# afiaka87/clip-guided-diffusion

Measured on AMD Instinct MI355X. Metric: diffusion steps/sec (UNet+CLIP+grad) at 256x256 cutn=16, higher is better.
Workload: dtype bf16x3 (split-bf16 MFMA, fp32 accumulate, fp32 storage); 1 GPU; BASELINE configs[1]: 256x256 class-cond UNet (554M), respace 250, cutn 16, batch 1/GPU, CLIP ViT-B/32, cgs 1000 tv 150 range 50, randomize_class, p_sample; global_batch=1, world_size_checked=1, collectives=none (single process)

## Files before the change

### clip-guided-diffusion_amd/csrc/capi.hip

```cpp
#include "../../include/cgd_mi355x.h"
#include "common.h"
#include "guidance.h"
#include "kernels.h"
#include "mfma_stage.h"

#define S(stream) ((hipStream_t)(stream))

extern "C" {

const char* cgd_version(void) { return "cgd_mi355x 0.1 (gfx950)"; }

int cgd_ctx_create(cgd_ctx** out, int device) {
  if (!out) return -3;
  cgd_ctx* ctx = new cgd_ctx();
  ctx->device = device;
  int prev = -1;
  (void)hipGetDevice(&prev);
  if (hipSetDevice(device) != hipSuccess) {
    delete ctx;
    return -1;
  }
  struct Restore {
    int d;
    ~Restore() {
      if (d >= 0) (void)hipSetDevice(d);
    }
  } restore{prev};
  hipDeviceProp_t prop;
  if (hipGetDeviceProperties(&prop, device) == hipSuccess) {
    ctx->num_cu = prop.multiProcessorCount;
    if (std::string(prop.gcnArchName).find("gfx950") == std::string::npos) {
      fprintf(stderr, "cgd_mi355x: device %d is %s, this library is built for gfx950 only\n", device, prop.gcnArchName);
      delete ctx;
      return -4;
    }
  }
  if (const char* e = getenv("CGD_DEFER")) ctx->defer_mode = atoi(e);
  if (const char* e = getenv("CGD_HGEMM_VAR")) ctx->hgemm_var = atoi(e);
  if (const char* e = getenv("CGD_HGEMM_EPI")) ctx->hgemm_epi = atoi(e);
  if (const char* e = getenv("CGD_TILE_ORDER")) ctx->tile_order = atoi(e);
  if (const char* e = getenv("CGD_FUSE_GN")) sscanf(e, "%d,%d,%d,%d", &ctx->fuse_gn, &ctx->fuse_gn_max_m, &ctx->fuse_gn_min_m, &ctx->fuse_gn_skip_m);
  if (const char* e = getenv("CGD_FUSE_ACT")) ctx->fuse_act = atoi(e);
  if (const char* e = getenv("CGD_HCONV_W8")) ctx->hconv_w8 = atoi(e);
  if (const char* e = getenv("CGD_ATTN_X3")) ctx->attn_x3 = atoi(e);
  if (const char* e = getenv("CGD_ATTN_FLASH")) ctx->attn_flash = atoi(e);
  int wino_env_mode = -1;
  if (const char* e = getenv("CGD_WINO")) sscanf(e, "%d,%d", &wino_env_mode, &ctx->wino_min_m);
  if (const char* e = getenv("CGD_THIN")) ctx->thin_direct = atoi(e);
  if (const char* e = getenv("CGD_GEMV")) ctx->gemv_mode = atoi(e);
  if (const char* e = getenv("CGD_WINO_NC")) ctx->wino_nc = atoi(e);
  ctx->wino_nc_default = ctx->wino_nc;
  if (wino_env_mode >= 0) cgd_apply_wino_mode(ctx, wino_env_mode);
  if (const char* e = getenv("CGD_GN_EPI")) ctx->gn_epi = atoi(e);
  if (const char* e = getenv("CGD_HGEMM_KG")) ctx->hgemm_kg = atoi(e) < 0 || atoi(e) > 2 ? 1 : atoi(e);
  if (const char* e = getenv("CGD_HGEMM_TM96")) ctx->hgemm_tm96 = atoi(e);
  if (const char* e = getenv("CGD_NT")) ctx->weight_nt = atoi(e);
  if (const char* e = getenv("CGD_KGEMM")) sscanf(e, "%d,%d,%d,%d,%d", &ctx->kgemm_mode, &ctx->kgemm_max_m, &ctx->kgemm_var, &ctx->kgemm_big_m, &ctx->kgemm_big_n);
  if (const char* e = getenv("CGD_EMBED_FUSE")) ctx->embed_fuse = atoi(e);
  if (const char* e = getenv("CGD_KCONV")) sscanf(e, "%d,%d,%d,%d,%d,%d,%d", &ctx->kconv_mode, &ctx->kconv_max_m, &ctx->kconv_min_chunks, &ctx->kconv_tw8, &ctx->kconv_slots, &ctx->kconv_ring, &ctx->kconv_th16);
  if (const char* e = getenv("CGD_HCONV_SPLIT")) sscanf(e, "%d,%d", &ctx->hconv_slots, &ctx->hconv_min_chunks);
  if (ctx->kconv_min_chunks < 1) ctx->kconv_min_chunks = 1;
  if (ctx->hconv_min_chunks < 1) ctx->hconv_min_chunks = 1;
  if (const char* e = getenv("CGD_HCONV_SMALL")) sscanf(e, "%d,%d,%d", &ctx->hconv_small_m, &ctx->hconv_small_slots, &ctx->hconv_small_min_chunks);
  ctx->ws_bytes = (size_t)256 << 20;
  if (hipMalloc((void**)&ctx->ws, ctx->ws_bytes) != hipSuccess) {
    delete ctx;
    return -1;
  }
  *out = ctx;
  return 0;
}

void cgd_ctx_destroy(cgd_ctx* ctx) {
  if (!ctx) return;
  {
  DeviceScope dev_scope(ctx);
  if (ctx->ws) (void)hipFree(ctx->ws);
  cgd_frag_cache_clear(ctx);
  cgd_chanstats_clear(ctx);
  if (ctx->frag_tmp) (void)hipFree(ctx->frag_tmp);
  for (ProfRec& r : ctx->prof_recs) {
    (void)hipEventDestroy(r.a);
    (void)hipEventDestroy(r.b);
  }
  for (hipEvent_t e : ctx->prof_pool) (void)hipEventDestroy(e);
  }
  delete ctx;
}

const char* cgd_last_error(cgd_ctx* ctx) { return ctx ? ctx->err.c_str() : "null context"; }

#define CGD_NEED_CTX(ctx)   \
  if (!(ctx)) return -3;    \
  DeviceScope dev_scope__(ctx)

int cgd_set_precision(cgd_ctx* ctx, int mode) {
  CGD_NEED_CTX(ctx);
  if (mode < 0 || mode > 2) CGD_FAIL(ctx, "precision mode must be 0 (f32), 1 (bf16x3) or 2 (bf16)");
  ctx->precision = mode;
  return 0;
}
int cgd_get_precision(cgd_ctx* ctx) { return ctx ? ctx->precision : -3; }
int64_t cgd_ctx_device_allocs(cgd_ctx* ctx) { return ctx ? (int64_t)ctx->device_allocs : -3; }

int cgd_set_tiles(cgd_ctx* ctx, int large, int small) {
  CGD_NEED_CTX(ctx);
  ctx->tile_huge = large >= 1000000 ? large / 1000000 : ctx->tile_huge;
  ctx->tile_large = large % 1000000;
  ctx->tile_small = small;
  return 0;
}

int cgd_set_hgemm(cgd_ctx* ctx, int mode, int min_m, int min_chunks) {
  CGD_NEED_CTX(ctx);
  ctx->hgemm_mode = mode;
  if (min_m > 0) ctx->hgemm_min_m = min_m;
  if (min_chunks > 0) ctx->hgemm_min_chunks = min_chunks;
  return 0;
}

int cgd_profile(cgd_ctx* ctx, int enable) {
  CGD_NEED_CTX(ctx);
  ctx->prof_on = enable != 0;
  return 0;
}
// ... 259 lines not shown
namespace {
__global__ __launch_bounds__(256) void mfma_peak_kernel(float* out, int iters) {
  cgd_f32x16 acc[4];
  for (int a = 0; a < 4; ++a)
    for (int e = 0; e < 16; ++e) acc[a][e] = 0.f;
  cgd_bf16x8 x, y;
  for (int e = 0; e < 8; ++e) {
    x[e] = (__bf16)(float)((threadIdx.x * 7 + e) % 13 - 6);
    y[e] = (__bf16)(0.001f * (float)((threadIdx.x * 3 + e) % 11 - 5));
  }
  for (int it = 0; it < iters; ++it) {
#pragma unroll
    for (int r = 0; r < 3; ++r)
#pragma unroll
      for (int a = 0; a < 4; ++a) acc[a] = __builtin_amdgcn_mfma_f32_32x32x16_bf16(x, y, acc[a], 0, 0, 0);
  }
  float s = 0.f;
  for (int a = 0; a < 4; ++a)
    for (int e = 0; e < 16; ++e) s += acc[a][e];
  if (s == 12345.678f) out[blockIdx.x * blockDim.x + threadIdx.x] = s;
}
}
extern "C" {
int cgd_op_mfma_peak(cgd_ctx* ctx, int iters, double* flop_out, void* stream) {
  CGD_NEED_CTX(ctx);
  if (iters <= 0) CGD_FAIL(ctx, "cgd_op_mfma_peak: iters must be positive");
  const int blocks = ctx->num_cu;
  if (flop_out) *flop_out = 2.0 * 32 * 32 * 16 * 12.0 * iters * blocks * 4;
  CGD_LAUNCH(mfma_peak_kernel, dim3(blocks), dim3(256), 0, S(stream), ctx->ws, iters);
  CGD_HIP(ctx, hipGetLastError());
  return 0;
}
int cgd_op_new_pass(cgd_ctx* ctx) {
  CGD_NEED_CTX(ctx);
  ++ctx->stats_serial;
  return 0;
}
int64_t cgd_op_gn_stats_offset(int B, int HW, int C) { return (int64_t)cgd_gn_stats_offset(B, HW, C); }
int64_t cgd_op_gn_record_merges(cgd_ctx* ctx) { return ctx ? (int64_t)ctx->gn_record_merges : -3; }
int cgd_set_wino(cgd_ctx* ctx, int mode, int min_m) {
  CGD_NEED_CTX(ctx);
  if (mode < 0 || (mode > 3 && mode != 5)) CGD_FAIL(ctx, "cgd_set_wino: mode must be 0, 1, 2, 3 or 5");
  cgd_apply_wino_mode(ctx, mode);
  if (min_m > 0) ctx->wino_min_m = min_m;
  return 0;
}
int cgd_set_hconv(cgd_ctx* ctx, int mode, int min_m) {
  CGD_NEED_CTX(ctx);
  ctx->hconv_mode = mode & 15;
  ctx->hconv_var = mode >> 4;
  ctx->hconv_min_m = min_m;
  return 0;
}
int cgd_op_conv3x3(cgd_ctx* ctx, const float* x, int ldx, const float* w, const float* w_frag, float* y, int ldy, const float* bias,
                   const float* R, int ldr, int Bn, int H, int W, int Cin, int Cout, int ups, int force_tile, int splitk, void* stream) {
  CGD_NEED_CTX(ctx);
  GemmParams p;
  p.Bpk = w_frag;
  p.A = x; p.lda = ldx; p.B = w; p.ldb = 9 * Cin; p.C = y; p.ldc = ldy; p.bias = bias; p.R = R; p.ldr = ldr;
  p.M = Bn * H * W; p.N = Cout; p.conv = 1; p.H = H; p.W = W; p.Cin = Cin; p.ups = ups; p.force_tile = force_tile; p.splitk = splitk;
  return cgd_launch_gemm(ctx, p, S(stream));
}
int cgd_op_conv_in(cgd_ctx* ctx, const float* x, const float* w, const float* bias, float* y, int Bn, int H, int W, int Cin, int Cout,
                   void* stream) {
  CGD_NEED_CTX(ctx);
  return cgd_launch_conv_in(ctx, x, w, bias, y, Bn, H, W, Cin, Cout, S(stream));
}
int cgd_op_conv_thin_out(cgd_ctx* ctx, const float* x, int ldx, const float* w, const float* bias, float* y, int Bn, int H, int W,
                         int Cin, int Cout, void* stream) {
  CGD_NEED_CTX(ctx);
  return cgd_launch_conv_thin_out(ctx, x, ldx, w, bias, y, Bn, H, W, Cin, Cout, S(stream));
}
int64_t cgd_op_gn_scratch_floats(int B, int HW, int C) { return (int64_t)cgd_gn_scratch_floats(B, HW, C); }
int cgd_op_gn_fwd(cgd_ctx* ctx, const float* x, int ldx, float* y, int ldy, int B, int HW, int C, const float* gamma, const float* beta,
                  const float* film, int act, float eps, float* scratch, void* stream) {
  CGD_NEED_CTX(ctx);
  return cgd_launch_gn_fwd(ctx, x, ldx, y, ldy, B, HW, C, gamma, beta, film, 2 * C, act, eps, scratch, S(stream));
}
int cgd_op_gn_bwd(cgd_ctx* ctx, const float* x, int ldx, const float* dz, int lddz, float* dx, int lddx, const float* add, int ldadd,
                  int B, int HW, int C, int act, float* scratch, void* stream) {
  CGD_NEED_CTX(ctx);
  return cgd_launch_gn_bwd(ctx, x, ldx, dz, lddz, dx, lddx, add, ldadd, B, HW, C, act, scratch, S(stream));
}
int cgd_op_ln_fwd(cgd_ctx* ctx, const float* x, float* y, int rows, int C, const float* gamma, const float* beta, float eps, float* stats,
                  void* stream) {
  CGD_NEED_CTX(ctx);
  return cgd_launch_ln_fwd(ctx, x, C, y, C, rows, C, gamma, beta, eps, stats, S(stream));
}
int cgd_op_ln_bwd(cgd_ctx* ctx, const float* x, const float* dy, float* dx, int rows, int C, const float* gamma, const float* stats,
                  void* stream) {
  CGD_NEED_CTX(ctx);
  return cgd_launch_ln_bwd(ctx, x, C, dy, C, dx, C, nullptr, 0, rows, C, gamma, stats, S(stream));
}
int cgd_op_pool2x2(cgd_ctx* ctx, const float* in, float* out, int B, int Ho, int Wo, int C, float scale, void* stream) {
  CGD_NEED_CTX(ctx);
  return cgd_launch_pool2x2(ctx, in, C, out, C, nullptr, 0, B, Ho, Wo, C, scale, S(stream));
}
int cgd_op_upsample2x(cgd_ctx* ctx, const float* in, float* out, int B, int Ho, int Wo, int C, float scale, void* stream) {
  CGD_NEED_CTX(ctx);
  return cgd_launch_upsample2x(ctx, in, C, out, C, nullptr, 0, B, Ho, Wo, C, scale, S(stream));
}
int cgd_op_act(cgd_ctx* ctx, const float* x, const float* dy, float* out, int64_t n, int act, void* stream) {
  CGD_NEED_CTX(ctx);
  if (dy) return cgd_launch_act_bwd(ctx, x, dy, out, n, act, S(stream));
  return cgd_launch_act_fwd(ctx, x, out, n, act, S(stream));
}
int64_t cgd_op_attn_buf_floats(int nb, int heads, int T, int d, int which) {
  const int64_t Tp = attn_tp(T), C = (int64_t)heads * d;
  switch (which) {
    case 0: return (int64_t)nb * 3 * C * Tp;
    case 4: return (int64_t)nb * C * Tp;
    default: return (int64_t)nb * heads * T * Tp;
  }
}
int cgd_op_attn_fwd(cgd_ctx* ctx, const float* qkv, float* out, int nb, int heads, int T, int d, int legacy, float* bufs[5],
                    void* stream) {
  CGD_NEED_CTX(ctx);
  AttnShape sh{nb, heads, T, d, heads * d, legacy};
  AttnBufs bf{bufs[0], bufs[1], bufs[2], bufs[3], bufs[4]};
  return cgd_attn_fwd(ctx, sh, qkv, 3 * heads * d, out, heads * d, bf, S(stream));
}
int cgd_op_attn_fwd_causal(cgd_ctx* ctx, const float* qkv, float* out, int nb, int heads, int T, int d, float* bufs[5], void* stream) {
  CGD_NEED_CTX(ctx);
  AttnShape sh{nb, heads, T, d, heads * d, 0, 1};
  AttnBufs bf{bufs[0], bufs[1], bufs[2], bufs[3], bufs[4]};
  return cgd_attn_fwd(ctx, sh, qkv, 3 * heads * d, out, heads * d, bf, S(stream));
}
int cgd_op_attn_bwd(cgd_ctx* ctx, const float* qkv, const float* dout, float* dqkv, int nb, int heads, int T, int d, int legacy,
                    float* bufs[5], void* stream) {
  CGD_NEED_CTX(ctx);
  AttnShape sh{nb, heads, T, d, heads * d, legacy};
  AttnBufs bf{bufs[0], bufs[1], bufs[2], bufs[3], bufs[4]};
  return cgd_attn_bwd(ctx, sh, qkv, 3 * heads * d, dout, heads * d, dqkv, 3 * heads * d, bf, S(stream));
}
}

void cgd_apply_wino_mode(cgd_ctx* ctx, int mode) {
  if (mode < 0 || (mode > 3 && mode != 5)) mode = 1;
  ctx->wino_mode = mode == 5 ? 3 : mode;
  ctx->wino_nc = mode == 5 ? 3 : ctx->wino_nc_default;
}
```

### clip-guided-diffusion_amd/csrc/common.h

```cpp
#pragma once
#include <hip/hip_runtime.h>
#include <stdint.h>
#include <stdio.h>
#include <atomic>
#include <string>
#include <utility>
#include <vector>

inline std::atomic<unsigned long long> g_cgd_launches{0}, g_cgd_reduces{0};
#define CGD_LAUNCH(...)                                          \
  do {                                                           \
    g_cgd_launches.fetch_add(1, std::memory_order_relaxed);      \
    hipLaunchKernelGGL(__VA_ARGS__);                             \
  } while (0)

enum { CGD_PREC_F32 = 0, CGD_PREC_BF16X3 = 1, CGD_PREC_BF16 = 2 };

enum { CGD_PROF_GEMM = 0, CGD_PROF_HCONV = 1, CGD_PROF_GN = 2, CGD_PROF_WCONV = 3, CGD_PROF_KCONV = 4, CGD_PROF_WCONV_GNB = 5, CGD_PROF_KINDS = 6 };

struct ProfRec {
  hipEvent_t a = nullptr, b = nullptr;
  double flops = 0.0;
  int kind = 0;
  bool live = false;
};

struct SplitSrc {
  const float* ws = nullptr;
  const float* bias = nullptr;
  const float* R = nullptr;
  long stride = 0;
  int n = 0;
  int N = 0, ldr = 0;
  float alpha = 1.f;
};
struct PendingReduce {
  bool valid = false;
  SplitSrc src;
  float* C = nullptr;
  int ldc = 0, M = 0;
  hipStream_t stream = nullptr;
};

struct ChanStatsEntry {
  const float* C = nullptr;
  int ldc = 0, N = 0;
  long M = 0;
  float* buf = nullptr;
  size_t cap = 0;
  hipStream_t stream = nullptr;
  unsigned long long serial = 0;
  int kind = 0;
};
struct ChanSrc {
  const float* p0 = nullptr;
  const float* p1 = nullptr;
  int n0 = 0, n1 = 0;
};

struct FragEntry {
  const float* w;
  int N, K, ldw;
  void* packed;
};

struct cgd_ctx {
  int device = 0;
  int precision = CGD_PREC_BF16X3;
  std::string err;
  float* ws = nullptr;
  size_t ws_bytes = 0;
  int num_cu = 256;
  int tile_huge = 1256, tile_large = 128, tile_small = 64;
  int hconv_var = 0;
  int hconv_small_m = 0, hconv_small_slots = 512, hconv_small_min_chunks = 2;
  int hconv_slots = 0, hconv_min_chunks = 4;
  int hconv_w8 = 0;
  int hconv_mode = 1, hconv_min_m = 256;
  int embed_fuse = 1;
  int gemv_mode = 1;
  int thin_direct = 1;
  int kconv_tw8 = 1;
  int kconv_th16 = 0;
  int kconv_ring = 2;
  int kconv_slots = 0;
  int kconv_mode = 1, kconv_max_m = 1024, kconv_min_chunks = 4;
  int wino_mode = 1, wino_min_m = 16384;
  int wino_nc_default = 0;
  int wino_nc = 0;
  int attn_x3 = 1;
  int attn_flash = 3;
  int fuse_act = 1;
  int fuse_gn_skip_m = 0;
  int fuse_gn_max_m = 1 << 30, fuse_gn_min_m = 4096;
  int fuse_gn = 1;
  int tile_order = 0;
  int hgemm_epi = 1;
  int hgemm_kg = 1;
  int weight_nt = 0;
  int kgemm_var = 0;
  int kgemm_big_m = 0, kgemm_big_n = 0;
  int kgemm_mode = 2, kgemm_max_m = 256;
  int hgemm_tm96 = 1;
  int hgemm_var = 1;
  int hgemm_mode = 1, hgemm_min_m = 64, hgemm_min_chunks = 4;
  PendingReduce pending;
  int defer_mode = 2;
  std::vector<ChanStatsEntry> chanstats;
  std::vector<float*> chanstats_retired;
  unsigned long long stats_serial = 1;
  unsigned long long device_allocs = 0;
  unsigned long long gn_record_merges = 0;
  bool last_wconv_bstat = false;
  int gn_epi = 3;
  std::vector<std::pair<const float*, int>> attn_fwd_path;
  std::vector<FragEntry> frag_cache;
  void* frag_tmp = nullptr;
  size_t frag_tmp_bytes = 0;
  bool prof_on = false;
  std::vector<ProfRec> prof_recs;
  std::vector<hipEvent_t> prof_pool;
  double prof_ms[CGD_PROF_KINDS] = {}, prof_flops[CGD_PROF_KINDS] = {}, prof_n[CGD_PROF_KINDS] = {};
};

struct ExactScope {
  cgd_ctx* ctx;
  int saved;
  explicit ExactScope(cgd_ctx* c) : ctx(c), saved(c->precision) { c->precision = CGD_PREC_F32; }
  ~ExactScope() { ctx->precision = saved; }
};

struct DeviceScope {
  int prev = -1;
  bool switched = false;
  explicit DeviceScope(const cgd_ctx* c) {
    if (c && hipGetDevice(&prev) == hipSuccess && prev != c->device) switched = hipSetDevice(c->device) == hipSuccess;
  }
  ~DeviceScope() {
    if (switched) (void)hipSetDevice(prev);
  }
};

int cgd_prof_fold(cgd_ctx* ctx, size_t keep_last);
int cgd_prof_begin(cgd_ctx* ctx, ProfRec* pr, int kind, double work, hipStream_t s);
int cgd_prof_stamp(cgd_ctx* ctx, ProfRec* pr, hipStream_t s);
void cgd_prof_push(cgd_ctx* ctx, ProfRec* pr);

#define CGD_HIP(ctx, expr)                                                                   \
  do {                                                                                       \
    hipError_t e__ = (expr);                                                                 \
    if (e__ != hipSuccess) {                                                                 \
      (ctx)->err = std::string(#expr) + ": " + hipGetErrorString(e__) + " @" + __FILE__ + ":" + \
                   std::to_string(__LINE__);                                                 \
      return -1;                                                                             \
    }                                                                                        \
  } while (0)

#define CGD_FAIL(ctx, msg)        \
  do {                            \
    (ctx)->err = (msg);           \
    return -2;                    \
  } while (0)

#define CGD_TRY(expr)             \
  do {                            \
    int r__ = (expr);             \
    if (r__ != 0) return r__;     \
  } while (0)

static inline int cdiv(long a, long b) { return (int)((a + b - 1) / b); }
static inline int grid_for(long n, int cap = 1024) {
  const int g = cdiv(n, 256);
  return g < cap ? g : cap;
}

struct GemmParams {
  const float* A = nullptr;
// ... 89 lines not shown
```

### clip-guided-diffusion_amd/csrc/elem.hip

```cpp
#include "common.h"
#include "kernels.h"

namespace {

__global__ __launch_bounds__(256) void pool2x2_kernel(const float* __restrict__ in, int ldi, float* __restrict__ out, int ldo,
                                                      const float* __restrict__ add, int ldadd, int B, int Ho, int Wo, int C,
                                                      float scale) {
  const int cq = C >> 2;
  const long total = (long)B * Ho * Wo * cq;
  for (long i = (long)blockIdx.x * blockDim.x + threadIdx.x; i < total; i += (long)gridDim.x * blockDim.x) {
    const int q = (int)(i % cq);
    const long pix = i / cq;
    const int x = (int)(pix % Wo);
    const long t = pix / Wo;
    const int y = (int)(t % Ho), b = (int)(t / Ho);
    const long Wi = 2L * Wo;
    const float* p00 = in + (((long)b * 2 * Ho + 2 * y) * Wi + 2 * x) * ldi + q * 4;
    const float4 a = *(const float4*)p00, c = *(const float4*)(p00 + ldi);
    const float4 d = *(const float4*)(p00 + Wi * ldi), e = *(const float4*)(p00 + Wi * ldi + ldi);
    float4 o = make_float4((a.x + c.x + d.x + e.x) * scale, (a.y + c.y + d.y + e.y) * scale, (a.z + c.z + d.z + e.z) * scale,
                           (a.w + c.w + d.w + e.w) * scale);
    if (add) {
      const float4 r = *(const float4*)(add + pix * ldadd + q * 4);
      o.x += r.x; o.y += r.y; o.z += r.z; o.w += r.w;
    }
    *(float4*)(out + pix * ldo + q * 4) = o;
  }
}

__global__ __launch_bounds__(256) void upsample2x_kernel(const float* __restrict__ in, int ldi, float* __restrict__ out, int ldo,
                                                         const float* __restrict__ add, int ldadd, int B, int Ho, int Wo, int C,
                                                         float scale) {
  const int cq = C >> 2;
  const long total = (long)B * Ho * Wo * cq;
  for (long i = (long)blockIdx.x * blockDim.x + threadIdx.x; i < total; i += (long)gridDim.x * blockDim.x) {
    const int q = (int)(i % cq);
    const long pix = i / cq;
    const int x = (int)(pix % Wo);
    const long t = pix / Wo;
    const int y = (int)(t % Ho), b = (int)(t / Ho);
    const float4 a = *(const float4*)(in + (((long)b * (Ho >> 1) + (y >> 1)) * (Wo >> 1) + (x >> 1)) * ldi + q * 4);
    float4 o = make_float4(a.x * scale, a.y * scale, a.z * scale, a.w * scale);
    if (add) {
      const float4 r = *(const float4*)(add + pix * ldadd + q * 4);
      o.x += r.x; o.y += r.y; o.z += r.z; o.w += r.w;
    }
    *(float4*)(out + pix * ldo + q * 4) = o;
  }
}

struct ResamplePair {
  const float* in[2];
  float* out[2];
  int ldi[2], ldo[2];
};
template <int UP>
__global__ __launch_bounds__(256) void resample2x_pair_kernel(const ResamplePair pp, int B, int Ho, int Wo, int C, float scale) {
  const int w = blockIdx.y;
  const float* __restrict__ in = pp.in[w];
  float* __restrict__ out = pp.out[w];
  const int ldi = pp.ldi[w], ldo = pp.ldo[w];
  const int cq = C >> 2;
  const long total = (long)B * Ho * Wo * cq;
  for (long i = (long)blockIdx.x * blockDim.x + threadIdx.x; i < total; i += (long)gridDim.x * blockDim.x) {
    const int q = (int)(i % cq);
    const long pix = i / cq;
    const int x = (int)(pix % Wo);
    const long t = pix / Wo;
    const int y = (int)(t % Ho), b = (int)(t / Ho);
    float4 o;
    if (UP) {
      const float4 a = *(const float4*)(in + (((long)b * (Ho >> 1) + (y >> 1)) * (Wo >> 1) + (x >> 1)) * ldi + q * 4);
      o = make_float4(a.x * scale, a.y * scale, a.z * scale, a.w * scale);
    } else {
      const long Wi = 2L * Wo;
      const float* p00 = in + (((long)b * 2 * Ho + 2 * y) * Wi + 2 * x) * ldi + q * 4;
      const float4 a = *(const float4*)p00, c = *(const float4*)(p00 + ldi);
      const float4 d = *(const float4*)(p00 + Wi * ldi), e = *(const float4*)(p00 + Wi * ldi + ldi);
      o = make_float4((a.x + c.x + d.x + e.x) * scale, (a.y + c.y + d.y + e.y) * scale, (a.z + c.z + d.z + e.z) * scale,
                      (a.w + c.w + d.w + e.w) * scale);
    }
    *(float4*)(out + pix * ldo + q * 4) = o;
  }
}

__global__ __launch_bounds__(256) void copy2d_kernel(const float* __restrict__ a, int lda, const float* __restrict__ b, int ldb,
                                                     float* __restrict__ out, int ldo, long rows, int C) {
  const int cq = C >> 2;
  const long total = rows * cq;
  for (long i = (long)blockIdx.x * blockDim.x + threadIdx.x; i < total; i += (long)gridDim.x * blockDim.x) {
    const int q = (int)(i % cq);
    const long r = i / cq;
    float4 o = *(const float4*)(a + r * lda + q * 4);
    if (b) {
      const float4 v = *(const float4*)(b + r * ldb + q * 4);
      o.x += v.x; o.y += v.y; o.z += v.z; o.w += v.w;
    }
    *(float4*)(out + r * ldo + q * 4) = o;
  }
}

__global__ __launch_bounds__(256) void concat2_kernel(const float* __restrict__ a, int lda, int Ca, const float* __restrict__ b, int ldb,
                                                      int Cb, float* __restrict__ out, int ldo, long rows) {
  const int qa = Ca >> 2, cq = (Ca + Cb) >> 2;
  const long total = rows * cq;
  for (long i = (long)blockIdx.x * blockDim.x + threadIdx.x; i < total; i += (long)gridDim.x * blockDim.x) {
    const int q = (int)(i % cq);
    const long r = i / cq;
    const float4 v = q < qa ? *(const float4*)(a + r * lda + q * 4) : *(const float4*)(b + r * ldb + (q - qa) * 4);
    *(float4*)(out + r * ldo + q * 4) = v;
  }
}

__device__ __forceinline__ float act_f(float u, int act) {
  if (act == 3) return 0.5f * u * (1.f + erff(u * 0.70710678f));
  const float k = act == 2 ? 1.702f : 1.f;
  return u / (1.f + __expf(-k * u));
}
__device__ __forceinline__ float dact_f(float u, int act) {
  if (act == 3) return 0.5f * (1.f + erff(u * 0.70710678f)) + u * 0.3989422804f * __expf(-0.5f * u * u);
  const float k = act == 2 ? 1.702f : 1.f;
  const float s = 1.f / (1.f + __expf(-k * u));
  return s * (1.f + k * u * (1.f - s));
}

__global__ __launch_bounds__(256) void act_fwd_kernel(const float* __restrict__ x, float* __restrict__ y, long n, int act) {
  for (long i = (long)blockIdx.x * blockDim.x + threadIdx.x; i < n; i += (long)gridDim.x * blockDim.x) y[i] = act_f(x[i], act);
}
__global__ __launch_bounds__(256) void act_bwd_kernel(const float* __restrict__ x, const float* __restrict__ dy,
                                                      float* __restrict__ dx, long n, int act) {
  for (long i = (long)blockIdx.x * blockDim.x + threadIdx.x; i < n; i += (long)gridDim.x * blockDim.x)
    dx[i] = dy[i] * dact_f(x[i], act);
}

__global__ void transpose_kernel(const float* __restrict__ in, int ldi, long si, float* __restrict__ out, int ldo, long so, int R,
                                 int Cc) {
  __shared__ float tile[32][33];
  in += (long)blockIdx.z * si;
  out += (long)blockIdx.z * so;
  const int c0 = blockIdx.x * 32, r0 = blockIdx.y * 32;
  for (int j = threadIdx.y; j < 32; j += 8) {
    const int r = r0 + j, c = c0 + threadIdx.x;
    tile[j][threadIdx.x] = (r < R && c < Cc) ? in[(long)r * ldi + c] : 0.f;
  }
  __syncthreads();
  for (int j = threadIdx.y; j < 32; j += 8) {
    const int c = c0 + j, r = r0 + threadIdx.x;
    if (c < Cc && r < ldo) out[(long)c * ldo + r] = tile[threadIdx.x][j];
  }
}

__global__ void timestep_embedding_kernel(const float* __restrict__ t, const float* __restrict__ freqs, float* __restrict__ out,
                                          int dim) {
  const int b = blockIdx.x, half = dim / 2;
  for (int i = threadIdx.x; i < half; i += blockDim.x) {
    const float a = t[b] * freqs[i];
    out[(long)b * dim + i] = cosf(a);
    out[(long)b * dim + half + i] = sinf(a);
  }
}

__global__ void embedding_add_kernel(const float* __restrict__ table, const int64_t* __restrict__ idx, float* __restrict__ out,
                                     int dim) {
  const int b = blockIdx.x;
  const float* row = table + idx[b] * dim;
  for (int i = threadIdx.x; i < dim; i += blockDim.x) out[(long)b * dim + i] += row[i];
}

__global__ __launch_bounds__(256) void vit_tokens_kernel(const float* __restrict__ patch, const float* __restrict__ cls,
                                                         const float* __restrict__ pos, float* __restrict__ tok, int N, int L,
                                                         int W) {
  const long total = (long)N * L * W;
  for (long i = (long)blockIdx.x * blockDim.x + threadIdx.x; i < total; i += (long)gridDim.x * blockDim.x) {
    const int w = (int)(i % W);
    const long t = i / W;
    const int l = (int)(t % L), n = (int)(t / L);
    const float v = l == 0 ? cls[w] : patch[((long)n * (L - 1) + (l - 1)) * W + w];
    tok[i] = v + pos[(long)l * W + w];
  }
}

__global__ __launch_bounds__(256) void patchify_kernel(float* img, float* cols, int N, int res, int P, int dir) {
  const int g = res / P;
  const long total = (long)N * 3 * res * res;
  for (long i = (long)blockIdx.x * blockDim.x + threadIdx.x; i < total; i += (long)gridDim.x * blockDim.x) {
    const int X = (int)(i % res);
    long t = i / res;
    const int Y = (int)(t % res);
    t /= res;
    const int c = (int)(t % 3), n = (int)(t / 3);
    const long ci = ((long)n * g * g + (Y / P) * g + (X / P)) * (3L * P * P) + (long)c * P * P + (Y % P) * P + (X % P);
    if (dir == 0)
      cols[ci] = img[i];
    else
      img[i] = cols[ci];
  }
}

__global__ __launch_bounds__(256) void fill_kernel(float* __restrict__ p, long n, float v) {
  for (long i = (long)blockIdx.x * blockDim.x + threadIdx.x; i < n; i += (long)gridDim.x * blockDim.x) p[i] = v;
}

inline int elem_grid(long n) { return grid_for(n, 4096); }

}

int cgd_launch_pool2x2(cgd_ctx* ctx, const float* in, int ldi, float* out, int ldo, const float* add, int ldadd, int B, int Ho,
                       int Wo, int C, float scale, hipStream_t s) {
  CGD_TRY(cgd_sync_pending(ctx, s));
  if ((C & 3) || (ldi & 3) || (ldo & 3)) CGD_FAIL(ctx, "pool2x2: C and strides must be multiples of 4");
  if (((uintptr_t)in | (uintptr_t)out | (uintptr_t)add) & 15) CGD_FAIL(ctx, "pool2x2: in / out / add must be 16-byte aligned");
  cgd_chanstats_invalidate(ctx, out, (long)B * Ho * Wo, ldo, C);
  CGD_LAUNCH(pool2x2_kernel, dim3(elem_grid((long)B * Ho * Wo * (C / 4))), dim3(256), 0, s, in, ldi, out, ldo, add, ldadd, B,
                     Ho, Wo, C, scale);
  CGD_HIP(ctx, hipGetLastError());
  return 0;
}

int cgd_launch_upsample2x(cgd_ctx* ctx, const float* in, int ldi, float* out, int ldo, const float* add, int ldadd, int B, int Ho,
                          int Wo, int C, float scale, hipStream_t s) {
  CGD_TRY(cgd_sync_pending(ctx, s));
  if ((C & 3) || (ldi & 3) || (ldo & 3)) CGD_FAIL(ctx, "upsample2x: C and strides must be multiples of 4");
  if (((uintptr_t)in | (uintptr_t)out | (uintptr_t)add) & 15) CGD_FAIL(ctx, "upsample2x: in / out / add must be 16-byte aligned");
  cgd_chanstats_invalidate(ctx, out, (long)B * Ho * Wo, ldo, C);
  CGD_LAUNCH(upsample2x_kernel, dim3(elem_grid((long)B * Ho * Wo * (C / 4))), dim3(256), 0, s, in, ldi, out, ldo, add, ldadd,
                     B, Ho, Wo, C, scale);
  CGD_HIP(ctx, hipGetLastError());
  return 0;
}

int cgd_launch_resample2x_pair(cgd_ctx* ctx, int up, const float* in0, int ldi0, float* out0, int ldo0, const float* in1, int ldi1, float* out1,
                               int ldo1, int B, int Ho, int Wo, int C, float scale, hipStream_t s) {
  CGD_TRY(cgd_sync_pending(ctx, s));
  if ((C & 3) || ((ldi0 | ldo0 | ldi1 | ldo1) & 3)) CGD_FAIL(ctx, "resample2x_pair: C and strides must be multiples of 4");
  cgd_chanstats_invalidate(ctx, out0, (long)B * Ho * Wo, ldo0, C);
  cgd_chanstats_invalidate(ctx, out1, (long)B * Ho * Wo, ldo1, C);
  ResamplePair pp;
  pp.in[0] = in0; pp.in[1] = in1; pp.out[0] = out0; pp.out[1] = out1;
  pp.ldi[0] = ldi0; pp.ldi[1] = ldi1; pp.ldo[0] = ldo0; pp.ldo[1] = ldo1;
  const dim3 grid(elem_grid((long)B * Ho * Wo * (C / 4)), 2);
  if (up)
    CGD_LAUNCH((resample2x_pair_kernel<1>), grid, dim3(256), 0, s, pp, B, Ho, Wo, C, scale);
  else
    CGD_LAUNCH((resample2x_pair_kernel<0>), grid, dim3(256), 0, s, pp, B, Ho, Wo, C, scale);
  CGD_HIP(ctx, hipGetLastError());
  return 0;
}

int cgd_launch_copy2d(cgd_ctx* ctx, const float* a, int lda, const float* b, int ldb, float* out, int ldo, long rows, int C,
                      hipStream_t s) {
  CGD_TRY(cgd_sync_pending(ctx, s));
  if ((C & 3) || (lda & 3) || (ldo & 3) || (b && (ldb & 3))) CGD_FAIL(ctx, "copy2d: C and strides must be multiples of 4");
  cgd_chanstats_invalidate(ctx, out, rows, ldo, C);
  CGD_LAUNCH(copy2d_kernel, dim3(elem_grid(rows * (C / 4))), dim3(256), 0, s, a, lda, b, ldb, out, ldo, rows, C);
  CGD_HIP(ctx, hipGetLastError());
  return 0;
}

int cgd_launch_concat2(cgd_ctx* ctx, const float* a, int lda, int Ca, const float* b, int ldb, int Cb, float* out, int ldo, long rows,
                       hipStream_t s) {
  CGD_TRY(cgd_sync_pending(ctx, s));
  if ((Ca & 3) || (Cb & 3) || (lda & 3) || (ldb & 3) || (ldo & 3)) CGD_FAIL(ctx, "concat2: channels and strides must be multiples of 4");
  cgd_chanstats_invalidate(ctx, out, rows, ldo, Ca + Cb);
  CGD_LAUNCH(concat2_kernel, dim3(elem_grid(rows * ((Ca + Cb) / 4))), dim3(256), 0, s, a, lda, Ca, b, ldb, Cb, out, ldo, rows);
  CGD_HIP(ctx, hipGetLastError());
  return 0;
}

static void flat_invalidate(cgd_ctx* ctx, const float* p, long n) {
  const long full = n >> 20, rest = n & ((1L << 20) - 1);
  if (full > 0) cgd_chanstats_invalidate(ctx, p, full, 1 << 20, 1 << 20);
  if (rest > 0) cgd_chanstats_invalidate(ctx, p + (full << 20), 1, (int)rest, (int)rest);
}

int cgd_launch_act_fwd(cgd_ctx* ctx, const float* x, float* y, long n, int act, hipStream_t s) {
  if (act < 1 || act > 3) CGD_FAIL(ctx, "activation code must be 1 (SiLU), 2 (QuickGELU) or 3 (GELU)");
  CGD_TRY(cgd_sync_pending(ctx, s));
  flat_invalidate(ctx, y, n);
  CGD_LAUNCH(act_fwd_kernel, dim3(elem_grid(n)), dim3(256), 0, s, x, y, n, act);
  CGD_HIP(ctx, hipGetLastError());
  return 0;
}
int cgd_launch_act_bwd(cgd_ctx* ctx, const float* x, const float* dy, float* dx, long n, int act, hipStream_t s) {
  if (act < 1 || act > 3) CGD_FAIL(ctx, "activation code must be 1 (SiLU), 2 (QuickGELU) or 3 (GELU)");
  CGD_TRY(cgd_sync_pending(ctx, s));
  flat_invalidate(ctx, dx, n);
  CGD_LAUNCH(act_bwd_kernel, dim3(elem_grid(n)), dim3(256), 0, s, x, dy, dx, n, act);
  CGD_HIP(ctx, hipGetLastError());
  return 0;
}

int cgd_launch_transpose(cgd_ctx* ctx, const float* in, int ldi, long si, float* out, int ldo, long so, int R, int Cc, int nb,
                         hipStream_t s) {
  CGD_TRY(cgd_sync_pending(ctx, s));
  CGD_LAUNCH(transpose_kernel, dim3(cdiv(Cc, 32), cdiv(ldo, 32), nb), dim3(32, 8), 0, s, in, ldi, si, out, ldo, so, R, Cc);
  CGD_HIP(ctx, hipGetLastError());
  return 0;
}

int cgd_launch_timestep_embedding(cgd_ctx* ctx, const float* t, const float* freqs, float* out, int B, int dim, hipStream_t s) {
  CGD_LAUNCH(timestep_embedding_kernel, dim3(B), dim3(128), 0, s, t, freqs, out, dim);
  CGD_HIP(ctx, hipGetLastError());
  return 0;
}

int cgd_launch_embedding_add(cgd_ctx* ctx, const float* table, const int64_t* idx, float* out, int B, int dim, hipStream_t s) {
  CGD_LAUNCH(embedding_add_kernel, dim3(B), dim3(256), 0, s, table, idx, out, dim);
  CGD_HIP(ctx, hipGetLastError());
  return 0;
}

int cgd_launch_vit_tokens(cgd_ctx* ctx, const float* patch, const float* cls, const float* pos, float* tok, int N, int L, int W,
                          hipStream_t s) {
  CGD_LAUNCH(vit_tokens_kernel, dim3(elem_grid((long)N * L * W)), dim3(256), 0, s, patch, cls, pos, tok, N, L, W);
  CGD_HIP(ctx, hipGetLastError());
  return 0;
}

int cgd_launch_patchify(cgd_ctx* ctx, const float* img, float* cols, int N, int res, int P, hipStream_t s) {
  CGD_LAUNCH(patchify_kernel, dim3(elem_grid((long)N * 3 * res * res)), dim3(256), 0, s, (float*)img, cols, N, res, P, 0);
  CGD_HIP(ctx, hipGetLastError());
  return 0;
}
int cgd_launch_unpatchify(cgd_ctx* ctx, const float* cols, float* img, int N, int res, int P, hipStream_t s) {
  CGD_LAUNCH(patchify_kernel, dim3(elem_grid((long)N * 3 * res * res)), dim3(256), 0, s, img, (float*)cols, N, res, P, 1);
  CGD_HIP(ctx, hipGetLastError());
  return 0;
}

int cgd_launch_fill(cgd_ctx* ctx, float* p, long n, float v, hipStream_t s) {
  CGD_LAUNCH(fill_kernel, dim3(elem_grid(n)), dim3(256), 0, s, p, n, v);
// ... 4 lines not shown
```

### clip-guided-diffusion_amd/csrc/kernels.h

```cpp
#pragma once
#include "common.h"

size_t cgd_gn_scratch_floats(int B, int HW, int C);
int cgd_launch_gn_fwd(cgd_ctx* ctx, const float* x, int ldx, float* y, int ldy, int B, int HW, int C, const float* gamma,
                      const float* beta, const float* film, int ldfilm, int act, float eps, float* scratch, hipStream_t s);
const float* cgd_gn_ab(const float* scratch, int B, int HW, int C);
const float* cgd_gn_coef(const float* scratch, int B, int HW, int C);
size_t cgd_gn_stats_offset(int B, int HW, int C);
int cgd_launch_gn_bwd(cgd_ctx* ctx, const float* x, int ldx, const float* dz, int lddz, float* dx, int lddx, const float* add,
                      int ldadd, int B, int HW, int C, int act, float* scratch, hipStream_t s, const float* add2 = nullptr,
                      int ldadd2 = 0);
int cgd_launch_ln_fwd(cgd_ctx* ctx, const float* x, int ldx, float* y, int ldy, int rows, int C, const float* gamma,
                      const float* beta, float eps, float* stats, hipStream_t s);
int cgd_launch_ln_bwd(cgd_ctx* ctx, const float* x, int ldx, const float* dy, int lddy, float* dx, int lddx, const float* add,
                      int ldadd, int rows, int C, const float* gamma, const float* stats, hipStream_t s);

int cgd_launch_pool2x2(cgd_ctx* ctx, const float* in, int ldi, float* out, int ldo, const float* add, int ldadd, int B, int Ho,
                       int Wo, int C, float scale, hipStream_t s);
int cgd_launch_resample2x_pair(cgd_ctx* ctx, int up, const float* in0, int ldi0, float* out0, int ldo0, const float* in1, int ldi1, float* out1,
                               int ldo1, int B, int Ho, int Wo, int C, float scale, hipStream_t s);
int cgd_launch_upsample2x(cgd_ctx* ctx, const float* in, int ldi, float* out, int ldo, const float* add, int ldadd, int B, int Ho,
                          int Wo, int C, float scale, hipStream_t s);
int cgd_launch_copy2d(cgd_ctx* ctx, const float* a, int lda, const float* b, int ldb, float* out, int ldo, long rows, int C,
                      hipStream_t s);
int cgd_launch_concat2(cgd_ctx* ctx, const float* a, int lda, int Ca, const float* b, int ldb, int Cb, float* out, int ldo, long rows,
                       hipStream_t s);
int cgd_launch_act_fwd(cgd_ctx* ctx, const float* x, float* y, long n, int act, hipStream_t s);
int cgd_launch_act_bwd(cgd_ctx* ctx, const float* x, const float* dy, float* dx, long n, int act, hipStream_t s);
int cgd_launch_transpose(cgd_ctx* ctx, const float* in, int ldi, long si, float* out, int ldo, long so, int R, int Cc, int nb,
                         hipStream_t s);
int cgd_launch_timestep_embedding(cgd_ctx* ctx, const float* t, const float* freqs, float* out, int B, int dim, hipStream_t s);
int cgd_launch_embedding_add(cgd_ctx* ctx, const float* table, const int64_t* idx, float* out, int B, int dim, hipStream_t s);
int cgd_launch_vit_tokens(cgd_ctx* ctx, const float* patch, const float* cls, const float* pos, float* tok, int N, int L, int W,
                          hipStream_t s);
int cgd_launch_patchify(cgd_ctx* ctx, const float* img, float* cols, int N, int res, int P, hipStream_t s);
int cgd_launch_unpatchify(cgd_ctx* ctx, const float* cols, float* img, int N, int res, int P, hipStream_t s);
int cgd_launch_fill(cgd_ctx* ctx, float* p, long n, float v, hipStream_t s);

int cgd_launch_softmax_rows(cgd_ctx* ctx, float* S, long rows, int T, int ld, hipStream_t s);
int cgd_launch_softmax_bwd_rows(cgd_ctx* ctx, const float* P, float* dP, long rows, int T, int ld, hipStream_t s);

struct AttnShape {
  int nb;
  int heads;
  int T;
  int d;
  int C;
  int legacy;
  int causal;
};
struct AttnBufs {
  float* qkvT;
  float* P;
  float* Pt;
  float* dP;
  float* dAt;
};
static inline int attn_tp(int T) { return (T + 3) & ~3; }
size_t cgd_attn_buf_floats(const cgd_ctx* ctx, const AttnShape& sh, int ldq, int ldo, int which);
int cgd_attn_fwd(cgd_ctx* ctx, const AttnShape& sh, const float* qkv, int ldq, float* out, int ldo, const AttnBufs& bufs,
                 hipStream_t s);
int cgd_attn_bwd(cgd_ctx* ctx, const AttnShape& sh, const float* qkv, int ldq, const float* dout, int lddo, float* dqkv, int lddq,
                 const AttnBufs& bufs, hipStream_t s);

int cgd_attn_flash_fwd(cgd_ctx* ctx, const AttnShape& sh, const float* qkv, int ldq, float* out, int ldo, const AttnBufs& bufs, long qo,
                       long ko, long vo, long step, hipStream_t s);
int cgd_attn_flash_bwd(cgd_ctx* ctx, const AttnShape& sh, const float* qkv, int ldq, const float* dout, int lddo, float* dqkv, int lddq,
                       const AttnBufs& bufs, long qo, long ko, long vo, long step, hipStream_t s);

struct CutoutGeom {
  int oy, ox, h, w;
};
int cgd_launch_cutouts_fwd(cgd_ctx* ctx, const float* x_in , const int* coords ,
                           float* out, int B, int H, int W, int cutn, int cs, int layout, int P, hipStream_t s);
int cgd_launch_cutouts_bwd(cgd_ctx* ctx, const float* dout, const int* coords, float* G , int B, int H, int W, int cutn,
                           int cs, int layout, int P, int accumulate, hipStream_t s);
int cgd_launch_cutouts_aug_fwd(cgd_ctx* ctx, const float* x_in, const int* coords, const float* params, const float* noise,
                               const int64_t* noise_off, float* out, int B, int H, int W, int cutn, int cs, int layout, int P,
                               hipStream_t s);
int cgd_launch_cutouts_aug_bwd(cgd_ctx* ctx, const float* dout, const int* coords, const float* params, float* G, float* scratch, int B,
                               int H, int W, int cutn, int cs, int layout, int P, int accumulate, hipStream_t s);
size_t cgd_cutouts_aug_scratch(int B, int H, int W, int cutn);
int cgd_aug_sample_map(const float* params, int h, int w, int32_t* affine_src, int32_t* persp_idx, float* persp_w);
int cgd_launch_cutouts_resize_fwd(cgd_ctx* ctx, const float* x_in, const int* coords, const int* flags, float* out, int B, int H, int W,
                                  int cutn, int cs, int layout, int P, hipStream_t s);
int cgd_launch_cutouts_resize_bwd(cgd_ctx* ctx, const float* dout, const int* coords, const int* flags, float* G, float* scratch, int B,
                                  int H, int W, int cutn, int cs, int layout, int P, int accumulate, hipStream_t s);
size_t cgd_cutouts_resize_scratch(int B, int H, int W, int cutn);
int cgd_resize_weights(int n, int m, float* w, int32_t* left, int* taps);
struct cgd_mask_coef;
int cgd_launch_masked_merge(cgd_ctx* ctx, float* sample, float* x0, const float* init, const float* mask, const float* n_known,
                            const float* n_re, float* x_re, int B, int H, int W, int init_batch, int mask_batch, int mask_channels,
                            const cgd_mask_coef& k, hipStream_t s);
struct cgd_reverse_coef;
int cgd_launch_ddim_reverse_update(cgd_ctx* ctx, const float* x, const float* out6, const float* init, float* x_next, float* x0,
                                   float* noise_out, int B, int H, int W, int init_batch, const cgd_reverse_coef& k, hipStream_t s);
int cgd_launch_spherical_loss(cgd_ctx* ctx, const float* emb, const float* targets, const float* weights, float* demb,
                              float* loss_part, int cutn, int B, int P, int D, float scale, hipStream_t s);

struct AttnPoolShape {
  int B, S2, C, d, out;
  int weight;
};
struct AttnPoolWeights {
  const float* posT;
// ... 16 lines not shown
```

### clip-guided-diffusion_amd/csrc/norm.hip

```cpp
#include "common.h"
#include "mfma_stage.h"
#include "kernels.h"

namespace {

constexpr int MAXJ = 4;
constexpr int GN_U = 4;

struct ColMap {
  int cq, TQ, rows, r, q0;
  bool active;
};
__device__ __forceinline__ ColMap col_map(int C) {
  ColMap m;
  m.cq = C >> 2;
  m.TQ = m.cq < 256 ? m.cq : 256;
  m.rows = 256 / m.TQ;
  m.r = threadIdx.x / m.TQ;
  m.q0 = threadIdx.x % m.TQ;
  m.active = m.r < m.rows;
  return m;
}

__device__ __forceinline__ float silu_f(float u) { return u / (1.f + __expf(-u)); }
// ... 211 lines not shown
  const int c = g * cpg + ci;
  const bool on = ci < cpg;
  const bool first = c < cs.n0;
  const float* base = first ? cs.p0 + ((long)b * ntile * cs.n0 + c) * 2 : cs.p1 + ((long)b * ntile * cs.n1 + (c - cs.n0)) * 2;
  const long rstride = (first ? cs.n0 : cs.n1) * 2L;
  constexpr int U = 8;
  double sum = 0.0;
  if (on)
    for (int t0 = tr; t0 < ntile; t0 += U * tstep) {
      float v[U];
#pragma unroll
      for (int u = 0; u < U; ++u) {
        const int t = t0 + u * tstep;
        v[u] = base[(t < ntile ? t : tr) * rstride];
      }
#pragma unroll
      for (int u = 0; u < U; ++u)
        if (t0 + u * tstep < ntile) sum += (double)v[u];
    }
  const double items = (double)ntile * cpg;
  const double mean = block_sum256(sum, red) / items;
  double m2 = 0.0;
  if (on)
    for (int t0 = tr; t0 < ntile; t0 += U * tstep) {
      float2 v[U];
#pragma unroll
      for (int u = 0; u < U; ++u) {
        const int t = t0 + u * tstep;
        v[u] = *(const float2*)(base + (t < ntile ? t : tr) * rstride);
      }
#pragma unroll
      for (int u = 0; u < U; ++u)
        if (t0 + u * tstep < ntile) {
          const double d = (double)v[u].x - mean;
          m2 += (double)v[u].y + 128.0 * d * d;
        }
    }
  m2 = block_sum256(m2, red);
  const double var = m2 / (items * 128.0);
  gn_fold_group(b, g, lane, cpg, (float)mean, (float)(1.0 / sqrt(var + (double)eps)), stats, gamma, beta, film, ldfilm, coef);
}

template <int ACT>
__global__ __launch_bounds__(256) void gn_apply_kernel(const float* __restrict__ x, int ldx, float* __restrict__ y, int ldy, int HW,
                                                       int C, int chunk, const float* __restrict__ coef) {
  const ColMap m = col_map(C);
  if (!m.active) return;
  const int b = blockIdx.y;
  const int p0 = blockIdx.x * chunk, p1 = min(HW, p0 + chunk);
  const float* xb = x + ((long)b * HW) * ldx;
  float* yb = y + ((long)b * HW) * ldy;
  for (int j = 0; j < MAXJ; ++j) {
    const int q = m.q0 + j * m.TQ;
    if (q >= m.cq) break;
    const float4* cf = (const float4*)(coef + ((long)b * C + q * 4) * 4);
    const float4 c0 = cf[0], c1 = cf[1], c2 = cf[2], c3 = cf[3];
    for (int pb = p0 + m.r; pb < p1; pb += GN_U * m.rows) {
      float4 vv[GN_U];
#pragma unroll
      for (int u = 0; u < GN_U; ++u) {
        const int p = pb + u * m.rows;
        vv[u] = *(const float4*)(xb + (long)(p < p1 ? p : pb) * ldx + q * 4);
      }
#pragma unroll
      for (int u = 0; u < GN_U; ++u) {
        const int p = pb + u * m.rows;
        if (p < p1) {
          const float4 v = vv[u];
          float4 o;
          o.x = v.x * c0.x + c0.y;
          o.y = v.y * c1.x + c1.y;
          o.z = v.z * c2.x + c2.y;
          o.w = v.w * c3.x + c3.y;
          if (ACT == 1) {
            o.x = silu_f(o.x); o.y = silu_f(o.y); o.z = silu_f(o.z); o.w = silu_f(o.w);
          }
          *(float4*)(yb + (long)p * ldy + q * 4) = o;
        }
      }
    }
  }
}

template <int ACT>
__global__ __launch_bounds__(256) void gn_bwd_partial_kernel(const float* __restrict__ x, int ldx, const float* dz, float* dzw,
                                                             int lddz, int HW, int C, int chunk, const float* __restrict__ coef,
                                                             float* __restrict__ part , const SplitSrc src) {
  __shared__ float lds_1[1024 * 4], lds_2[1024 * 4];
  __shared__ float red_1[256 * 4], red_2[256 * 4];
  const ColMap m = col_map(C);
  const int b = blockIdx.y, ck = blockIdx.x, nchunk = gridDim.x;
  const int p0 = ck * chunk, p1 = min(HW, p0 + chunk);
  const float* xb = x + ((long)b * HW) * ldx;
  const float* db = dz + ((long)b * HW) * lddz;
  const int cpg = C / 32;
  for (int j = 0; j < MAXJ; ++j) {
    const int q = m.q0 + j * m.TQ;
    if (q >= m.cq) break;
    const float4* cf = (const float4*)(coef + ((long)b * C + q * 4) * 4);
    const float4 c0 = cf[0], c1 = cf[1], c2 = cf[2], c3 = cf[3];
    float4 s1 = make_float4(0, 0, 0, 0), s2 = make_float4(0, 0, 0, 0);
    if (m.active) {
      for (int pb = p0 + m.r; pb < p1; pb += GN_U * m.rows) {
       float4 vv[GN_U], dd[GN_U];
#pragma unroll
       for (int u = 0; u < GN_U; ++u) {
         const int p = pb + u * m.rows, pc = p < p1 ? p : pb;
         vv[u] = *(const float4*)(xb + (long)pc * ldx + q * 4);
         if (src.n) {
           dd[u] = split_load4(src, (long)b * HW + pc, q * 4);
           if (p < p1) *(float4*)(dzw + ((long)b * HW + pc) * lddz + q * 4) = dd[u];
         } else {
           dd[u] = *(const float4*)(db + (long)pc * lddz + q * 4);
         }
       }
#pragma unroll
       for (int u = 0; u < GN_U; ++u) {
        if (pb + u * m.rows >= p1) continue;
        const float4 v = vv[u];
        float4 d = dd[u];
        if (ACT == 1) {
          d.x *= dsilu_f(v.x * c0.x + c0.y);
          d.y *= dsilu_f(v.y * c1.x + c1.y);
          d.z *= dsilu_f(v.z * c2.x + c2.y);
          d.w *= dsilu_f(v.w * c3.x + c3.y);
        }
        s1.x += d.x; s1.y += d.y; s1.z += d.z; s1.w += d.w;
        s2.x += d.x * (v.x - c0.w); s2.y += d.y * (v.y - c1.w); s2.z += d.z * (v.z - c2.w); s2.w += d.w * (v.w - c3.w);
       }
      }
    }
    if (m.rows > 1) {
      if (m.active) {
        *(float4*)&red_1[(m.r * m.cq + q) * 4] = s1;
        *(float4*)&red_2[(m.r * m.cq + q) * 4] = s2;
      }
      __syncthreads();
      if (m.r == 0) {
        for (int rr = 1; rr < m.rows; ++rr) {
          const float4 a = *(const float4*)&red_1[(rr * m.cq + q) * 4];
          const float4 c = *(const float4*)&red_2[(rr * m.cq + q) * 4];
          s1.x += a.x; s1.y += a.y; s1.z += a.z; s1.w += a.w;
          s2.x += c.x; s2.y += c.y; s2.z += c.z; s2.w += c.w;
        }
      }
    }
    if (m.r == 0) {
      s1.x *= c0.z; s1.y *= c1.z; s1.z *= c2.z; s1.w *= c3.z;
      s2.x *= c0.z; s2.y *= c1.z; s2.z *= c2.z; s2.w *= c3.z;
      *(float4*)&lds_1[q * 4] = s1;
      *(float4*)&lds_2[q * 4] = s2;
    }
  }
  __syncthreads();
  if (threadIdx.x < 32) {
    const int g = threadIdx.x;
    float a = 0.f, c2 = 0.f;
    for (int c = g * cpg; c < (g + 1) * cpg; ++c) {
      a += lds_1[c];
      c2 += lds_2[c];
    }
    float* o = part + (((long)b * nchunk + ck) * 32 + g) * 2;
    o[0] = a;
    o[1] = c2;
  }
}

__global__ __launch_bounds__(256) void gn_bwd_coef_kernel(const float* __restrict__ part, int nchunk, const float* __restrict__ stats,
                                                          const float* __restrict__ coef, int C, int HW, float* __restrict__ bcoef) {
  __shared__ double red[4];
  const int b = blockIdx.y, g = blockIdx.x, lane = threadIdx.x;
  const int cpg = C / 32;
  double p1 = 0.0, p2 = 0.0;
  for (int ck = lane; ck < nchunk; ck += 256) {
    const float2 v = *(const float2*)(part + (((long)b * nchunk + ck) * 32 + g) * 2);
    p1 += v.x;
    p2 += v.y;
  }
  p1 = block_sum256(p1, red);
  p2 = block_sum256(p2, red);
  const double N = (double)HW * cpg;
  const float rstd = stats[((long)b * 32 + g) * 2 + 1];
  const float a2 = (float)((double)rstd * rstd * rstd * p2 / N), a3 = (float)((double)rstd * p1 / N);
  for (int c = g * cpg + lane; c < (g + 1) * cpg; c += 256) {
    float* o = bcoef + ((long)b * C + c) * 4;
    o[0] = rstd * coef[((long)b * C + c) * 4 + 2];
    o[1] = a2;
    o[2] = a3;
    o[3] = 0.f;
  }
}

__global__ __launch_bounds__(256) void gn_bwd_coef_ch_kernel(const float* __restrict__ rec, int ntile, int lg, const float* __restrict__ stats,
                                                             const float* __restrict__ coef, int C, int HW, float* __restrict__ bcoef) {
  __shared__ double red[4];
  const int b = blockIdx.y, g = blockIdx.x, lane = threadIdx.x;
  const int cpg = C / 32;
  const int ci = lane & ((1 << lg) - 1), tr = lane >> lg, tstep = 256 >> lg;
  const bool on = ci < cpg;
  const float* base = rec + ((long)b * ntile * C + g * cpg + ci) * 2;
  const long rstride = 2L * C;
  constexpr int U = 8;
  double p1 = 0.0, p2 = 0.0;
  if (on)
    for (int t0 = tr; t0 < ntile; t0 += U * tstep) {
      float2 v[U];
#pragma unroll
      for (int u = 0; u < U; ++u) {
        const int t = t0 + u * tstep;
        v[u] = *(const float2*)(base + (t < ntile ? t : tr) * rstride);
      }
#pragma unroll
      for (int u = 0; u < U; ++u)
        if (t0 + u * tstep < ntile) {
          p1 += (double)v[u].x;
          p2 += (double)v[u].y;
        }
    }
  p1 = block_sum256(p1, red);
  p2 = block_sum256(p2, red);
  const double N = (double)HW * cpg;
  const float rstd = stats[((long)b * 32 + g) * 2 + 1];
  const float a2 = (float)((double)rstd * rstd * rstd * p2 / N), a3 = (float)((double)rstd * p1 / N);
  for (int c = g * cpg + lane; c < (g + 1) * cpg; c += 256) {
    float* o = bcoef + ((long)b * C + c) * 4;
    o[0] = rstd * coef[((long)b * C + c) * 4 + 2];
    o[1] = a2;
    o[2] = a3;
    o[3] = 0.f;
  }
}

__device__ __forceinline__ float4 gn_ld4_nt(const float* p) {
  const cgd_f32x4 v = cgd_ld16_nt<cgd_f32x4>(p);
  return make_float4(v.x, v.y, v.z, v.w);
}
__device__ __forceinline__ void gn_st4_nt(float* p, const float4 o) {
  cgd_st16_nt(p, cgd_f32x4{o.x, o.y, o.z, o.w});
}
template <int ACT>
__global__ __launch_bounds__(256) void gn_bwd_apply_kernel(const float* __restrict__ x, int ldx, const float* __restrict__ dz,
                                                           int lddz, float* __restrict__ dx, int lddx, const float* __restrict__ add,
                                                           int ldadd, const float* __restrict__ add2, int ldadd2, int HW, int C, int chunk,
                                                           const float* __restrict__ coef, const float* __restrict__ bcoef) {
  const ColMap m = col_map(C);
  if (!m.active) return;
  const int b = blockIdx.y;
  const int p0 = blockIdx.x * chunk, p1 = min(HW, p0 + chunk);
  const float* xb = x + ((long)b * HW) * ldx;
  const float* db = dz + ((long)b * HW) * lddz;
  float* ob = dx + ((long)b * HW) * lddx;
  const float* ab = add ? add + ((long)b * HW) * ldadd : nullptr;
  const float* ab2 = add2 ? add2 + ((long)b * HW) * ldadd2 : nullptr;
  for (int j = 0; j < MAXJ; ++j) {
    const int q = m.q0 + j * m.TQ;
    if (q >= m.cq) break;
    const float4* cf = (const float4*)(coef + ((long)b * C + q * 4) * 4);
    const float4* bf = (const float4*)(bcoef + ((long)b * C + q * 4) * 4);
    const float4 c0 = cf[0], c1 = cf[1], c2 = cf[2], c3 = cf[3];
    const float4 b0 = bf[0], b1 = bf[1], b2 = bf[2], b3 = bf[3];
    for (int pb = p0 + m.r; pb < p1; pb += GN_U * m.rows) {
     float4 vv[GN_U], dd[GN_U], aa[GN_U];
#pragma unroll
     for (int u = 0; u < GN_U; ++u) {
       const int p = pb + u * m.rows, pc = p < p1 ? p : pb;
       vv[u] = gn_ld4_nt(xb + (long)pc * ldx + q * 4);
       dd[u] = gn_ld4_nt(db + (long)pc * lddz + q * 4);
       if (ab) aa[u] = gn_ld4_nt(ab + (long)pc * ldadd + q * 4);
       if (ab2) {
         const float4 a2 = gn_ld4_nt(ab2 + (long)pc * ldadd2 + q * 4);
         if (ab) { aa[u].x += a2.x; aa[u].y += a2.y; aa[u].z += a2.z; aa[u].w += a2.w; } else aa[u] = a2;
       }
     }
#pragma unroll
     for (int u = 0; u < GN_U; ++u) {
      const int p = pb + u * m.rows;
      if (p >= p1) continue;
      const float4 v = vv[u];
      float4 d = dd[u];
      if (ACT == 1) {
        d.x *= dsilu_f(v.x * c0.x + c0.y);
        d.y *= dsilu_f(v.y * c1.x + c1.y);
        d.z *= dsilu_f(v.z * c2.x + c2.y);
        d.w *= dsilu_f(v.w * c3.x + c3.y);
      }
      float4 o;
      o.x = d.x * b0.x - (v.x - c0.w) * b0.y - b0.z;
      o.y = d.y * b1.x - (v.y - c1.w) * b1.y - b1.z;
      o.z = d.z * b2.x - (v.z - c2.w) * b2.y - b2.z;
      o.w = d.w * b3.x - (v.w - c3.w) * b3.y - b3.z;
      if (ab || ab2) {
        const float4 a = aa[u];
        o.x += a.x; o.y += a.y; o.z += a.z; o.w += a.w;
      }
      gn_st4_nt(ob + (long)p * lddx + q * 4, o);
     }
    }
  }
}

__global__ __launch_bounds__(256) void ln_fwd_generic_kernel(const float* __restrict__ x, int ldx, float* __restrict__ y, int ldy, int rows,
                                                     int C, const float* __restrict__ gamma, const float* __restrict__ beta,
                                                     float eps, float* __restrict__ stats ) {
  const int row = blockIdx.x * 4 + (threadIdx.x >> 6), lane = threadIdx.x & 63;
  if (row >= rows) return;
  const float* xr = x + (long)row * ldx;
  float s = 0.f;
  for (int c = lane; c < C; c += 64) s += xr[c];
  for (int o = 32; o > 0; o >>= 1) s += __shfl_xor(s, o, 64);
  const float mean = s / C;
  float v = 0.f;
  for (int c = lane; c < C; c += 64) {
    const float d = xr[c] - mean;
    v += d * d;
  }
  for (int o = 32; o > 0; o >>= 1) v += __shfl_xor(v, o, 64);
  const float rstd = rsqrtf(v / C + eps);
  float* yr = y + (long)row * ldy;
  for (int c = lane; c < C; c += 64) yr[c] = (xr[c] - mean) * rstd * gamma[c] + beta[c];
  if (lane == 0 && stats) {
    stats[row * 2] = mean;
    stats[row * 2 + 1] = rstd;
  }
}

__global__ __launch_bounds__(256) void ln_bwd_generic_kernel(const float* __restrict__ x, int ldx, const float* __restrict__ dy, int lddy,
                                                     float* __restrict__ dx, int lddx, const float* __restrict__ add, int ldadd,
                                                     int rows, int C, const float* __restrict__ gamma,
                                                     const float* __restrict__ stats) {
  const int row = blockIdx.x * 4 + (threadIdx.x >> 6), lane = threadIdx.x & 63;
  if (row >= rows) return;
  const float* xr = x + (long)row * ldx;
  const float* dr = dy + (long)row * lddy;
  const float mean = stats[row * 2], rstd = stats[row * 2 + 1];
  float s1 = 0.f, s2 = 0.f;
  for (int c = lane; c < C; c += 64) {
    const float g = dr[c] * gamma[c];
    s1 += g;
    s2 += g * (xr[c] - mean) * rstd;
  }
  for (int o = 32; o > 0; o >>= 1) {
    s1 += __shfl_xor(s1, o, 64);
    s2 += __shfl_xor(s2, o, 64);
  }
  s1 /= C;
  s2 /= C;
  float* orow = dx + (long)row * lddx;
  const float* ar = add ? add + (long)row * ldadd : nullptr;
  for (int c = lane; c < C; c += 64) {
    const float xh = (xr[c] - mean) * rstd;
    float o = rstd * (dr[c] * gamma[c] - s1 - xh * s2);
// ... 218 lines not shown
            s += d;
            ss += d * d;
          }
        }
      }
    }
  }
  s = block_sum(s, red);
  ss = block_sum(ss, red);
  const float ms = s / n;
  const float mean = k0 + ms, var = fmaxf(ss / n - ms * ms, 0.f);
  const float rstd = rsqrtf(var + eps);
  if (threadIdx.x == 0) {
    stats[((long)b * 32 + g) * 2] = mean;
    stats[((long)b * 32 + g) * 2 + 1] = rstd;
  }
  if (threadIdx.x < cpg) {
    const int c = g * cpg + threadIdx.x;
    float gm = gamma[c], bt = beta[c];
    if (film) {
      const float sc = 1.f + film[(long)b * ldfilm + c], sh = film[(long)b * ldfilm + C + c];
      gm *= sc;
      bt = bt * sc + sh;
    }
    float* o = coef + ((long)b * C + c) * 4;
    o[0] = ca[threadIdx.x] = gm * rstd;
    o[1] = cb[threadIdx.x] = bt - mean * gm * rstd;
    o[2] = gm;
    o[3] = mean;
    float* ab = coef + (long)gridDim.y * C * 8 + ((long)b * C + c) * 2;
    ab[0] = o[0];
    ab[1] = o[1];
  }
  if (!y) return;
  __syncthreads();
  if (!act_q) return;
  float a[VEC], bb[VEC];
#pragma unroll
  for (int e = 0; e < VEC; ++e) {
    a[e] = ca[q * VEC + e];
    bb[e] = cb[q * VEC + e];
  }
  if constexpr (CACHE) {
#pragma unroll
    for (int it = 0; it < 8; ++it) {
      const int p = r + it * rows;
      if (p < HW) {
        V o;
#pragma unroll
        for (int e = 0; e < VEC; ++e) {
          float t = vget<VEC>(vc[it], e) * a[e] + bb[e];
          if (ACT == 1) t = silu_f(t);
          vset<VEC>(o, e, t);
        }
        *(V*)(yg + (long)p * ldy) = o;
      }
    }
    return;
  }
  for (int p0 = r; p0 < HW; p0 += rows * GS_U) {
    V v[GS_U];
#pragma unroll
    for (int u = 0; u < GS_U; ++u) {
      const int p = p0 + u * rows;
      v[u] = *(const V*)(xg + (long)(p < HW ? p : r) * ldx);
    }
#pragma unroll
    for (int u = 0; u < GS_U; ++u) {
      const int p = p0 + u * rows;
      if (p < HW) {
        V o;
#pragma unroll
        for (int e = 0; e < VEC; ++e) {
          float t = vget<VEC>(v[u], e) * a[e] + bb[e];
          if (ACT == 1) t = silu_f(t);
          vset<VEC>(o, e, t);
        }
        *(V*)(yg + (long)p * ldy) = o;
      }
    }
  }
}

template <int ACT, int VEC, bool CACHE>
__global__ __launch_bounds__(GS_NT) void gn_small_bwd_kernel(const float* __restrict__ x, int ldx, const float* dz, float* dzw, int lddz,
                                                             float* dx, int lddx, const float* add, int ldadd, const float* add2, int ldadd2,
                                                             int HW, int C, int lg, const float* __restrict__ stats,
                                                             const float* __restrict__ coef, const SplitSrc src) {
  typedef typename VecT<VEC>::T V;
  __shared__ float red[GS_NT / 64];
  const int g = blockIdx.x, b = blockIdx.y, cpg = C / 32, cq = cpg / VEC, n = HW * cpg;
  const int q = threadIdx.x & ((1 << lg) - 1), r = threadIdx.x >> lg, rows = GS_NT >> lg;
  const bool act_q = q < cq;
  const int qc = act_q ? q : 0;
  const float* xg = x + (long)b * HW * ldx + g * cpg + qc * VEC;
  const float* dg = dz + (long)b * HW * lddz + g * cpg + qc * VEC;
  float* dwg = dzw + (long)b * HW * lddz + g * cpg + qc * VEC;
  const long row0 = (long)b * HW;
  const int col = g * cpg + qc * VEC;
  float* og = dx + (long)b * HW * lddx + g * cpg + qc * VEC;
  const float* ag = add ? add + (long)b * HW * ldadd + g * cpg + qc * VEC : nullptr;
  const float* ag2 = add2 ? add2 + (long)b * HW * ldadd2 + g * cpg + qc * VEC : nullptr;
  const float mean = stats[((long)b * 32 + g) * 2], rstd = stats[((long)b * 32 + g) * 2 + 1];
  float a[VEC], bb[VEC], gc[VEC];
#pragma unroll
  for (int e = 0; e < VEC; ++e) {
    const float* o = coef + ((long)b * C + g * cpg + qc * VEC + e) * 4;
    a[e] = o[0];
    bb[e] = o[1];
    gc[e] = o[2];
  }
  float p1 = 0.f, p2 = 0.f;
  V xc[CACHE ? 4 : 1], dc[CACHE ? 4 : 1];
  if constexpr (CACHE) {
#pragma unroll
    for (int it = 0; it < 4; ++it) {
      const int p = r + it * rows;
      if (act_q && p < HW) {
        xc[it] = *(const V*)(xg + (long)p * ldx);
        dc[it] = src.n ? split_load<VEC>(src, row0 + p, col) : *(const V*)(dg + (long)p * lddz);
      }
    }
#pragma unroll
    for (int it = 0; it < 4; ++it) {
      if (act_q && r + it * rows < HW) {
#pragma unroll
        for (int e = 0; e < VEC; ++e) {
          const float xe = vget<VEC>(xc[it], e);
          float du = vget<VEC>(dc[it], e);
          if (ACT == 1) du *= dsilu_f(xe * a[e] + bb[e]);
          du *= gc[e];
          vset<VEC>(dc[it], e, du);
          p1 += du;
          p2 += du * (xe - mean);
        }
      }
    }
  } else
  if (act_q) {
    for (int p0 = r; p0 < HW; p0 += rows * GS_U) {
      V xv[GS_U], dv[GS_U];
#pragma unroll
      for (int u = 0; u < GS_U; ++u) {
        const int p = p0 + u * rows, pc = p < HW ? p : r;
        xv[u] = *(const V*)(xg + (long)pc * ldx);
        if (src.n) {
          dv[u] = split_load<VEC>(src, row0 + pc, col);
          if (p < HW) *(V*)(dwg + (long)pc * lddz) = dv[u];
        } else {
          dv[u] = *(const V*)(dg + (long)pc * lddz);
        }
      }
#pragma unroll
      for (int u = 0; u < GS_U; ++u) {
        if (p0 + u * rows < HW) {
#pragma unroll
          for (int e = 0; e < VEC; ++e) {
            const float xe = vget<VEC>(xv[u], e);
            float du = vget<VEC>(dv[u], e);
            if (ACT == 1) du *= dsilu_f(xe * a[e] + bb[e]);
            du *= gc[e];
            p1 += du;
            p2 += du * (xe - mean);
          }
        }
      }
    }
  }
  p1 = block_sum(p1, red);
  p2 = block_sum(p2, red);
  if (!act_q) return;
  const float a2 = rstd * rstd * rstd * p2 / n, a3 = rstd * p1 / n;
  if constexpr (CACHE) {
    V av[4];
#pragma unroll
    for (int it = 0; it < 4; ++it) {
      const int p = r + it * rows;
      if (ag && p < HW) av[it] = *(const V*)(ag + (long)p * ldadd);
      if (ag2 && p < HW) {
        const V a2 = *(const V*)(ag2 + (long)p * ldadd2);
        if (ag) av[it] += a2; else av[it] = a2;
      }
    }
#pragma unroll
    for (int it = 0; it < 4; ++it) {
      const int p = r + it * rows;
      if (p < HW) {
        V o;
#pragma unroll
        for (int e = 0; e < VEC; ++e) {
          float t = vget<VEC>(dc[it], e) * rstd - (vget<VEC>(xc[it], e) - mean) * a2 - a3;
          if (ag || ag2) t += vget<VEC>(av[it], e);
          vset<VEC>(o, e, t);
        }
        *(V*)(og + (long)p * lddx) = o;
      }
    }
    return;
  }
  for (int p0 = r; p0 < HW; p0 += rows * GS_U) {
    V xv[GS_U], dv[GS_U], av[GS_U];
#pragma unroll
    for (int u = 0; u < GS_U; ++u) {
      const int p = p0 + u * rows, pc = p < HW ? p : r;
      xv[u] = *(const V*)(xg + (long)pc * ldx);
      dv[u] = *(const V*)(dg + (long)pc * lddz);
      if (ag) av[u] = *(const V*)(ag + (long)pc * ldadd);
      if (ag2) {
        const V a2 = *(const V*)(ag2 + (long)pc * ldadd2);
        if (ag) av[u] += a2; else av[u] = a2;
      }
    }
#pragma unroll
    for (int u = 0; u < GS_U; ++u) {
      const int p = p0 + u * rows;
      if (p < HW) {
        V o;
#pragma unroll
        for (int e = 0; e < VEC; ++e) {
          const float xe = vget<VEC>(xv[u], e);
          float du = vget<VEC>(dv[u], e);
          if (ACT == 1) du *= dsilu_f(xe * a[e] + bb[e]);
          float t = du * gc[e] * rstd - (xe - mean) * a2 - a3;
          if (ag || ag2) t += vget<VEC>(av[u], e);
          vset<VEC>(o, e, t);
        }
        *(V*)(og + (long)p * lddx) = o;
      }
    }
  }
}

template <int ACT>
void launch_gn_small_fwd(const float* x, int ldx, float* y, int ldy, int B, int HW, int C, const float* gamma, const float* beta,
                         const float* film, int ldfilm, float eps, float* stats, float* coef, hipStream_t s, const SplitSrc& src) {
  const int cpg = C / 32;
  const bool v4 = !(cpg & 3) && !(ldx & 3) && !(ldy & 3) && !(((uintptr_t)x | (uintptr_t)y) & 15) && !(src.n && ((src.N | src.ldr) & 3));
  const int cq = v4 ? cpg / 4 : cpg;
  int lg = 0;
  while ((1 << lg) < cq) ++lg;
  const bool cache = (long)HW <= 8L * (GS_NT >> lg) && !getenv("CGD_GN_NOCACHE");
#define GN_SF(V_, C_) CGD_LAUNCH((gn_small_fwd_kernel<ACT, V_, C_>), dim3(32, B), dim3(GS_NT), 0, s, x, (float*)x, ldx, y, ldy, HW, C, lg, gamma, beta, film, ldfilm, eps, stats, coef, src)
  if (v4) {
    if (cache) GN_SF(4, true); else GN_SF(4, false);
  } else {
    if (cache) GN_SF(1, true); else GN_SF(1, false);
  }
#undef GN_SF
}

template <int ACT>
void launch_gn_small_bwd(const float* x, int ldx, const float* dz, int lddz, float* dx, int lddx, const float* add, int ldadd,
                         const float* add2, int ldadd2, int B, int HW, int C, const float* stats, const float* coef, hipStream_t s,
                         const SplitSrc& src) {
  const int cpg = C / 32;
  const bool v4 = !(cpg & 3) && !(ldx & 3) && !(lddz & 3) && !(lddx & 3) && !(ldadd & 3) && !(ldadd2 & 3) &&
                  !(((uintptr_t)x | (uintptr_t)dz | (uintptr_t)dx | (uintptr_t)add | (uintptr_t)add2) & 15) && !(src.n && ((src.N | src.ldr) & 3));
  const int cq = v4 ? cpg / 4 : cpg;
  int lg = 0;
  while ((1 << lg) < cq) ++lg;
  const bool cache = (long)HW <= 4L * (GS_NT >> lg) && !getenv("CGD_GN_NOCACHE");
#define GN_SB(V_, C_) CGD_LAUNCH((gn_small_bwd_kernel<ACT, V_, C_>), dim3(32, B), dim3(GS_NT), 0, s, x, ldx, dz, (float*)dz, lddz, dx, lddx, add, ldadd, add2, ldadd2, HW, C, lg, stats, coef, src)
  if (v4) {
    if (cache) GN_SB(4, true); else GN_SB(4, false);
  } else {
    if (cache) GN_SB(1, true); else GN_SB(1, false);
  }
#undef GN_SB
}

static int gn_small_hw() {
  static int v = -1;
  if (v < 0) {
    const char* e = getenv("CGD_GN_SMALL_HW");
    v = e ? atoi(e) : 1024;
  }
  return v;
}
#define GN_SMALL_HW gn_small_hw()

int pick_chunk(int HW, int B) {
  int chunk = HW * B / 512;
  if (chunk < 8) chunk = 8;
  if (chunk > 256) chunk = 256;
  if ((HW + chunk - 1) / chunk > 2048) chunk = (HW + 2047) / 2048;
  if (chunk > HW) chunk = HW;
  return chunk;
}

}

size_t cgd_gn_scratch_floats(int B, int HW, int C) {
  const int chunk = pick_chunk(HW, B);
  const int nchunk = cdiv(HW, chunk);
  return (size_t)B * nchunk * 64 + (size_t)B * 64 + (size_t)B * C * 4 * 2 + (size_t)B * C * 2;
}

const float* cgd_gn_ab(const float* scratch, int B, int HW, int C) {
  const int nchunk = cdiv(HW, pick_chunk(HW, B));
  return scratch + (size_t)B * nchunk * 64 + (size_t)B * 64 + (size_t)B * C * 4 * 2;
}

size_t cgd_gn_stats_offset(int B, int HW, int C) {
  (void)C;
  return (size_t)B * cdiv(HW, pick_chunk(HW, B)) * 64;
}

const float* cgd_gn_coef(const float* scratch, int B, int HW, int C) {
  const int nchunk = cdiv(HW, pick_chunk(HW, B));
  return scratch + (size_t)B * nchunk * 64 + (size_t)B * 64;
}

static void gn_layout(float* scratch, int B, int HW, int C, int* chunk, int* nchunk, float** part, float** stats, float** coef,
                      float** bcoef) {
  *chunk = pick_chunk(HW, B);
  *nchunk = cdiv(HW, *chunk);
  *part = scratch;
  *stats = *part + (size_t)B * *nchunk * 64;
  *coef = *stats + (size_t)B * 64;
  *bcoef = *coef + (size_t)B * C * 4;
}

int cgd_launch_gn_fwd(cgd_ctx* ctx, const float* x, int ldx, float* y, int ldy, int B, int HW, int C, const float* gamma,
                      const float* beta, const float* film, int ldfilm, int act, float eps, float* scratch, hipStream_t s) {
  if (C % 32 || C > 4096) CGD_FAIL(ctx, "groupnorm: C must be a multiple of 32 and <= 4096");
  if ((ldx & 3) || (y && (ldy & 3))) CGD_FAIL(ctx, "groupnorm: row strides must be multiples of 4");
  if (HW > GN_SMALL_HW && (((uintptr_t)x | (uintptr_t)y) & 15)) CGD_FAIL(ctx, "groupnorm: x / y must be 16-byte aligned above the single-launch size");
  float* const y_written = y;
  const int ldy_written = ldy;
  if (!y) ldy = 4;
  int chunk, nchunk;
  float *part, *stats, *coef, *bcoef;
  gn_layout(scratch, B, HW, C, &chunk, &nchunk, &part, &stats, &coef, &bcoef);
  SplitSrc src;
  if (!((HW > GN_SMALL_HW || ctx->defer_mode >= 2) && cgd_take_pending(ctx, x, (long)B * HW, C, ldx, s, &src))) CGD_TRY(cgd_flush_pending(ctx, s));
  if (src.n && (((src.N | src.ldr) & 3) || ((uintptr_t)src.ws & 15) || ((uintptr_t)src.R & 15) || ((uintptr_t)src.bias & 15)) && HW > GN_SMALL_HW) {
    ctx->pending.valid = true; ctx->pending.src = src; ctx->pending.C = (float*)x; ctx->pending.ldc = ldx; ctx->pending.M = B * HW; ctx->pending.stream = s;
    CGD_TRY(cgd_flush_pending(ctx, s));
    src = SplitSrc();
  }
  ChanSrc cs;
  const bool epi = !src.n && HW > GN_SMALL_HW && !(HW & 127) && (ctx->gn_epi & 1) && cgd_chanstats_find(ctx, x, ldx, (long)B * HW, C, s, &cs);
  if (y_written) cgd_chanstats_invalidate(ctx, y_written, (long)B * HW, ldy_written, C);
  ProfRec pr;
  CGD_TRY(cgd_prof_begin(ctx, &pr, CGD_PROF_GN, ((y ? 8.0 : 4.0) + (src.n ? 4.0 * src.n : 0.0)) * B * HW * C, s));
  if (epi) {
    ++ctx->gn_record_merges;
    int lg = 0;
    while ((1 << lg) < C / 32) ++lg;
    CGD_LAUNCH(gn_stats_final_ch_kernel, dim3(32, B), dim3(256), 0, s, cs, HW / 128, C / 32, lg, eps, stats, gamma, beta, film, ldfilm, coef);
    if (y) {
      if (act)
        CGD_LAUNCH((gn_apply_kernel<1>), dim3(nchunk, B), dim3(256), 0, s, x, ldx, y, ldy, HW, C, chunk, coef);
      else
        CGD_LAUNCH((gn_apply_kernel<0>), dim3(nchunk, B), dim3(256), 0, s, x, ldx, y, ldy, HW, C, chunk, coef);
    }
    CGD_TRY(cgd_prof_stamp(ctx, &pr, s));
    cgd_prof_push(ctx, &pr);
    CGD_HIP(ctx, hipGetLastError());
    return 0;
  }
  if (HW <= GN_SMALL_HW) {
    if (act)
      launch_gn_small_fwd<1>(x, ldx, y, ldy, B, HW, C, gamma, beta, film, ldfilm, eps, stats, coef, s, src);
    else
      launch_gn_small_fwd<0>(x, ldx, y, ldy, B, HW, C, gamma, beta, film, ldfilm, eps, stats, coef, s, src);
    CGD_TRY(cgd_prof_stamp(ctx, &pr, s));
    cgd_prof_push(ctx, &pr);
    CGD_HIP(ctx, hipGetLastError());
    return 0;
  }
  CGD_LAUNCH(gn_stats_partial_kernel, dim3(nchunk, B), dim3(256), 0, s, x, (float*)x, ldx, HW, C, chunk, part, src);
  CGD_LAUNCH(gn_stats_final_kernel, dim3(32, B), dim3(256), 0, s, part, nchunk, HW, chunk, C / 32, eps, stats, gamma, beta, film,
                     ldfilm, coef);
  if (y) {
    if (act)
      CGD_LAUNCH((gn_apply_kernel<1>), dim3(nchunk, B), dim3(256), 0, s, x, ldx, y, ldy, HW, C, chunk, coef);
    else
      CGD_LAUNCH((gn_apply_kernel<0>), dim3(nchunk, B), dim3(256), 0, s, x, ldx, y, ldy, HW, C, chunk, coef);
  }
  CGD_TRY(cgd_prof_stamp(ctx, &pr, s));
  cgd_prof_push(ctx, &pr);
  CGD_HIP(ctx, hipGetLastError());
  return 0;
}

int cgd_launch_gn_bwd(cgd_ctx* ctx, const float* x, int ldx, const float* dz, int lddz, float* dx, int lddx, const float* add,
                      int ldadd, int B, int HW, int C, int act, float* scratch, hipStream_t s, const float* add2, int ldadd2) {
  if (C % 32 || C > 4096) CGD_FAIL(ctx, "groupnorm backward: C must be a multiple of 32 and <= 4096");
  if (HW > GN_SMALL_HW && (((ldx | lddz | lddx | (add ? ldadd : 0) | (add2 ? ldadd2 : 0)) & 3) ||
                           (((uintptr_t)x | (uintptr_t)dz | (uintptr_t)dx | (uintptr_t)add | (uintptr_t)add2) & 15)))
    CGD_FAIL(ctx, "groupnorm backward: above the single-launch size, row strides must be multiples of 4 and x / dz / dx / add 16-byte aligned");
  int chunk, nchunk;
  float *part, *stats, *coef, *bcoef;
  gn_layout(scratch, B, HW, C, &chunk, &nchunk, &part, &stats, &coef, &bcoef);
  SplitSrc src;
  if (!((HW > GN_SMALL_HW || ctx->defer_mode >= 2) && cgd_take_pending(ctx, dz, (long)B * HW, C, lddz, s, &src))) CGD_TRY(cgd_flush_pending(ctx, s));
  if (src.n && (((src.N | src.ldr) & 3) || ((uintptr_t)src.ws & 15) || ((uintptr_t)src.R & 15) || ((uintptr_t)src.bias & 15)) && HW > GN_SMALL_HW) {
    ctx->pending.valid = true; ctx->pending.src = src; ctx->pending.C = (float*)dz; ctx->pending.ldc = lddz; ctx->pending.M = B * HW; ctx->pending.stream = s;
    CGD_TRY(cgd_flush_pending(ctx, s));
    src = SplitSrc();
  }
  ProfRec pr;
  CGD_TRY(cgd_prof_begin(ctx, &pr, CGD_PROF_GN, (12.0 + (add ? 4.0 : 0.0) + (add2 ? 4.0 : 0.0) + (src.n ? 4.0 * src.n : 0.0)) * B * HW * C, s));
  if (HW <= GN_SMALL_HW) {
    if (act)
      launch_gn_small_bwd<1>(x, ldx, dz, lddz, dx, lddx, add, ldadd, add2, ldadd2, B, HW, C, stats, coef, s, src);
    else
      launch_gn_small_bwd<0>(x, ldx, dz, lddz, dx, lddx, add, ldadd, add2, ldadd2, B, HW, C, stats, coef, s, src);
    CGD_TRY(cgd_prof_stamp(ctx, &pr, s));
    cgd_prof_push(ctx, &pr);
    CGD_HIP(ctx, hipGetLastError());
    cgd_chanstats_invalidate(ctx, dx, (long)B * HW, lddx, C);
    return 0;
  }
  ChanSrc cs;
  const bool merged = !src.n && !(HW & 127) && (ctx->gn_epi & 2) && cgd_chanstats_find(ctx, dz, lddz, (long)B * HW, C, s, &cs, 1) && cs.n0 == C;
  cgd_chanstats_invalidate(ctx, dx, (long)B * HW, lddx, C);
  if (merged) {
    ++ctx->gn_record_merges;
    int lg = 0;
    while ((1 << lg) < C / 32) ++lg;
    CGD_LAUNCH(gn_bwd_coef_ch_kernel, dim3(32, B), dim3(256), 0, s, cs.p0, HW / 128, lg, stats, coef, C, HW, bcoef);
  } else {
    if (act) {
      CGD_LAUNCH((gn_bwd_partial_kernel<1>), dim3(nchunk, B), dim3(256), 0, s, x, ldx, dz, (float*)dz, lddz, HW, C, chunk, coef, part, src);
    } else {
      CGD_LAUNCH((gn_bwd_partial_kernel<0>), dim3(nchunk, B), dim3(256), 0, s, x, ldx, dz, (float*)dz, lddz, HW, C, chunk, coef, part, src);
    }
    CGD_LAUNCH(gn_bwd_coef_kernel, dim3(32, B), dim3(256), 0, s, part, nchunk, stats, coef, C, HW, bcoef);
  }
  if (act) {
    CGD_LAUNCH((gn_bwd_apply_kernel<1>), dim3(nchunk, B), dim3(256), 0, s, x, ldx, dz, lddz, dx, lddx, add, ldadd, add2, ldadd2, HW, C, chunk, coef, bcoef);
  } else {
    CGD_LAUNCH((gn_bwd_apply_kernel<0>), dim3(nchunk, B), dim3(256), 0, s, x, ldx, dz, lddz, dx, lddx, add, ldadd, add2, ldadd2, HW, C, chunk, coef, bcoef);
  }
  CGD_TRY(cgd_prof_stamp(ctx, &pr, s));
  cgd_prof_push(ctx, &pr);
  CGD_HIP(ctx, hipGetLastError());
  return 0;
}

int cgd_launch_ln_fwd(cgd_ctx* ctx, const float* x, int ldx, float* y, int ldy, int rows, int C, const float* gamma,
                      const float* beta, float eps, float* stats, hipStream_t s) {
  const bool vec = C % 256 == 0 && C <= 1024 && !(ldx & 3) && !(ldy & 3) && !(((uintptr_t)x | (uintptr_t)y | (uintptr_t)gamma | (uintptr_t)beta) & 15);
  const dim3 grid(cdiv(rows, 4)), blk(256);
  SplitSrc src;
  const bool slices_ok = vec && ctx->defer_mode >= 1;
  if (!(slices_ok && cgd_take_pending(ctx, x, rows, C, ldx, s, &src))) CGD_TRY(cgd_flush_pending(ctx, s));
  if (src.n && (((src.N | src.ldr) & 3) || ((uintptr_t)src.R & 15) || ((uintptr_t)src.bias & 15))) {
    ctx->pending.valid = true; ctx->pending.src = src; ctx->pending.C = (float*)x; ctx->pending.ldc = ldx; ctx->pending.M = rows; ctx->pending.stream = s;
    CGD_TRY(cgd_flush_pending(ctx, s));
    src = SplitSrc();
  }
  if (!vec) {
    CGD_LAUNCH(ln_fwd_generic_kernel, grid, blk, 0, s, x, ldx, y, ldy, rows, C, gamma, beta, eps, stats);
  } else {
    switch (C / 256) {
      case 1: CGD_LAUNCH((ln_fwd_kernel<1>), grid, blk, 0, s, x, (float*)x, ldx, y, ldy, rows, gamma, beta, eps, stats, src); break;
      case 2: CGD_LAUNCH((ln_fwd_kernel<2>), grid, blk, 0, s, x, (float*)x, ldx, y, ldy, rows, gamma, beta, eps, stats, src); break;
      case 3: CGD_LAUNCH((ln_fwd_kernel<3>), grid, blk, 0, s, x, (float*)x, ldx, y, ldy, rows, gamma, beta, eps, stats, src); break;
      default: CGD_LAUNCH((ln_fwd_kernel<4>), grid, blk, 0, s, x, (float*)x, ldx, y, ldy, rows, gamma, beta, eps, stats, src); break;
    }
  }
  CGD_HIP(ctx, hipGetLastError());
  return 0;
}

int cgd_launch_ln_bwd(cgd_ctx* ctx, const float* x, int ldx, const float* dy, int lddy, float* dx, int lddx, const float* add,
                      int ldadd, int rows, int C, const float* gamma, const float* stats, hipStream_t s) {
  const bool vec = C % 256 == 0 && C <= 1024 && !(ldx & 3) && !(lddy & 3) && !(lddx & 3) && !(ldadd & 3) &&
                   !(((uintptr_t)x | (uintptr_t)dy | (uintptr_t)dx | (uintptr_t)add | (uintptr_t)gamma) & 15);
  const dim3 grid(cdiv(rows, 4)), blk(256);
  SplitSrc src;
  const bool slices_ok = vec && ctx->defer_mode >= 1;
  if (!(slices_ok && cgd_take_pending(ctx, dy, rows, C, lddy, s, &src))) CGD_TRY(cgd_flush_pending(ctx, s));
  if (src.n && (((src.N | src.ldr) & 3) || ((uintptr_t)src.R & 15) || ((uintptr_t)src.bias & 15))) {
    ctx->pending.valid = true; ctx->pending.src = src; ctx->pending.C = (float*)dy; ctx->pending.ldc = lddy; ctx->pending.M = rows; ctx->pending.stream = s;
    CGD_TRY(cgd_flush_pending(ctx, s));
    src = SplitSrc();
  }
  if (!vec) {
    CGD_LAUNCH(ln_bwd_generic_kernel, grid, blk, 0, s, x, ldx, dy, lddy, dx, lddx, add, ldadd, rows, C, gamma, stats);
  } else {
    switch (C / 256) {
      case 1: CGD_LAUNCH((ln_bwd_kernel<1>), grid, blk, 0, s, x, ldx, dy, lddy, dx, lddx, add, ldadd, rows, gamma, stats, src); break;
      case 2: CGD_LAUNCH((ln_bwd_kernel<2>), grid, blk, 0, s, x, ldx, dy, lddy, dx, lddx, add, ldadd, rows, gamma, stats, src); break;
      case 3: CGD_LAUNCH((ln_bwd_kernel<3>), grid, blk, 0, s, x, ldx, dy, lddy, dx, lddx, add, ldadd, rows, gamma, stats, src); break;
      default: CGD_LAUNCH((ln_bwd_kernel<4>), grid, blk, 0, s, x, ldx, dy, lddy, dx, lddx, add, ldadd, rows, gamma, stats, src); break;
    }
  }
  CGD_HIP(ctx, hipGetLastError());
  return 0;
}

float* cgd_chanstats_register(cgd_ctx* ctx, const float* C, int ldc, int N, long M, hipStream_t s, int kind) {
  if ((M & 127) || (N & 3)) return nullptr;
  const size_t need = (size_t)(M / 128) * N * 2;
  ChanStatsEntry* e = nullptr;
  for (ChanStatsEntry& q : ctx->chanstats)
    if (q.C == C && q.kind == kind) e = &q;
  if (!e) {
    ctx->chanstats.emplace_back();
    e = &ctx->chanstats.back();
    e->C = C;
    e->kind = kind;
  }
  if (e->cap < need) {
    if (e->buf) ctx->chanstats_retired.push_back(e->buf);
    e->buf = nullptr;
    e->cap = 0;
    void* p = nullptr;
    if (hipMalloc(&p, need * sizeof(float)) != hipSuccess) {
      (void)hipGetLastError();
      e->serial = 0;
      return nullptr;
    }
    ++ctx->device_allocs;
    e->buf = (float*)p;
// ... 49 lines not shown
```

### clip-guided-diffusion_amd/csrc/unet.hip

```cpp
#include <cmath>
#include <memory>

#include "../../include/cgd_mi355x.h"
#include "net.h"

namespace {

__global__ void pack_conv3x3_kernel(const float* __restrict__ w, float* __restrict__ wf, float* __restrict__ wd, int Co, int Ci) {
  const long total = (long)Co * Ci * 9;
  for (long i = (long)blockIdx.x * blockDim.x + threadIdx.x; i < total; i += (long)gridDim.x * blockDim.x) {
    const int kx = (int)(i % 3);
    long t = i / 3;
    const int ky = (int)(t % 3);
    t /= 3;
    const int ci = (int)(t % Ci), co = (int)(t / Ci);
    const float v = w[i];
    if (wf) wf[((long)co * 9 + ky * 3 + kx) * Ci + ci] = v;
    if (wd) wd[((long)ci * 9 + (2 - ky) * 3 + (2 - kx)) * Co + co] = v;
  }
}

}

int cgd_pack_conv3x3(cgd_ctx* ctx, const float* w, float* wf, float* wd, int Co, int Ci, hipStream_t s) {
// ... 43 lines not shown
  int B = 0, T = 0;
  TV x;
  DevBuf n, qkv, a, out, sc, da, dqkv, dn, dx;
  AttnScratch att;
  int fwd(UNet& u, TV x, int B, int& H, int& W, TV* out, hipStream_t s) override;
  int bwd(UNet& u, TV dout, TV* din, hipStream_t s) override;
};

struct UNet : NetBase {
  int ensure_wino(ResBlock* rb, long pixels, hipStream_t s);
  cgd_unet_config cfg;
  bool encoder_only = false;
  int ted = 0, ch0 = 0, ch_last = 0;
  long emb_total = 0;
  std::vector<std::vector<std::unique_ptr<Module>>> in_blocks;
  std::vector<std::unique_ptr<Module>> mid;
  std::vector<std::vector<std::unique_ptr<Module>>> out_blocks;
  std::vector<int> in_chans;
  std::vector<int> in_ds;
  std::vector<ResBlock*> resblocks;
  float *stem_wf = 0, *stem_wd = 0, *head_wf = 0, *head_wd = 0;
  float *emb_w_all = 0, *emb_b_all = 0, *freqs = 0;
  int B = 0, H = 0, W = 0;
  bool have_fwd = false;
  int fwd_prec = 0;
  DevBuf temb, e1, e1s, e2, e2s, emb_all, h0, headn, head_s, dheadn, dhead;
  DevBuf emb_slot1;
  const float* emb_cur = nullptr;
  int emb_B[2] = {0, 0};
  std::vector<DevBuf> cats;
  std::vector<TV> hs;
  std::vector<std::pair<int, int>> hs_hw;
  std::vector<TV> cat_in;
  std::vector<int> cat_c1;
  std::vector<std::pair<int, int>> cat_hw;
  TV head_in;

  int build();
  int finalize(hipStream_t s);
  int embed(const float* t, const int64_t* y, int Bn, int slot, hipStream_t s, bool ahead = false);
  int forward(const float* x, const float* t, const int64_t* y, float* out, int B, int H, int W, hipStream_t s, int slot = -1);
  int dgrad(const float* gout, float* gx, hipStream_t s);
};

int UNet::ensure_wino(ResBlock* rb, long pixels, hipStream_t s) {
  if (rb->wino_ready && rb->wino_prec != ctx->precision) rb->wino_ready = false;
  if (!ctx->wino_mode || pixels < ctx->wino_min_m || rb->wino_ready) return 0;
  if (ctx->precision != CGD_PREC_BF16X3 && ctx->precision != CGD_PREC_F32) return 0;
  const std::string& p = rb->pre;
  if (!rb->cw1wp) CGD_TRY(alloc(&rb->cw1wp, cgd_wconv_packed_floats(rb->cout, rb->cin)));
  if (!rb->cw1wd) CGD_TRY(alloc(&rb->cw1wd, cgd_wconv_packed_floats(rb->cout, rb->cin)));
  if (!rb->cw2wp) CGD_TRY(alloc(&rb->cw2wp, cgd_wconv_packed_floats(rb->cout, rb->cout)));
  if (!rb->cw2wd) CGD_TRY(alloc(&rb->cw2wd, cgd_wconv_packed_floats(rb->cout, rb->cout)));
  CGD_TRY(cgd_pack_conv3x3_wino(ctx, P(p + ".in_layers.2.weight"), rb->cw1wp, rb->cout, rb->cin, 0, s));
  CGD_TRY(cgd_pack_conv3x3_wino(ctx, P(p + ".in_layers.2.weight"), rb->cw1wd, rb->cout, rb->cin, 1, s));
  CGD_TRY(cgd_pack_conv3x3_wino(ctx, P(p + ".out_layers.3.weight"), rb->cw2wp, rb->cout, rb->cout, 0, s));
  CGD_TRY(cgd_pack_conv3x3_wino(ctx, P(p + ".out_layers.3.weight"), rb->cw2wd, rb->cout, rb->cout, 1, s));
  rb->wino_ready = true;
  rb->wino_prec = ctx->precision;
  return 0;
}

int ResBlock::fwd(UNet& u, TV xin, int Bn, int& Hh, int& Ww, TV* o, hipStream_t s) {
  cgd_ctx* ctx = u.ctx;
  B = Bn; H = Hh; W = Ww;
  Ho = up ? 2 * H : (down ? H / 2 : H);
  Wo = up ? 2 * W : (down ? W / 2 : W);
  x = xin;
  const long npi = (long)B * H * W, npo = (long)B * Ho * Wo;
  CGD_TRY(u.ensure(s1, cgd_gn_scratch_floats(B, H * W, cin)));
  CGD_TRY(u.ensure(s2, cgd_gn_scratch_floats(B, Ho * Wo, cout)));
  CGD_TRY(u.ensure(h2, npo * cout));
  if (!dst.p) CGD_TRY(u.ensure(out, npo * cout));
  float* const outp = dst.p ? dst.p : out.p;
  const int ldo = dst.p ? dst.ld : cout;
  CGD_TRY(u.ensure_wino(this, npo, s));
  GemmParams c1;
  c1.B = cw1f; c1.Bpk = cw1fp; c1.Bwk = wino_ready ? cw1wp : nullptr; c1.bwk_prec = wino_prec; c1.ldb = 9 * cin; c1.C = h2.p; c1.ldc = cout; c1.bias = cb1;
  c1.M = (int)npo; c1.N = cout; c1.conv = 1; c1.H = Ho; c1.W = Wo; c1.Cin = cin; c1.ups = up ? 1 : 0;
  c1.defer = 1;
  c1.stats = 1;
  c1.A = x.p; c1.lda = x.ld;
  const bool fuse1 = !down && cgd_conv_uses_hconv(ctx, c1);
  const float* skip_src = x.p;
  int skip_ld = x.ld;
  if (fuse1) {
    CGD_TRY(cgd_launch_gn_fwd(ctx, x.p, x.ld, nullptr, 0, B, H * W, cin, g1, b1, nullptr, 0, 1, 1e-5f, s1.p, s));
    c1.gn_ab = cgd_gn_ab(s1.p, B, H * W, cin);
  } else {
    CGD_TRY(u.ensure(h1, npi * cin));
    CGD_TRY(cgd_launch_gn_fwd(ctx, x.p, x.ld, h1.p, cin, B, H * W, cin, g1, b1, nullptr, 0, 1, 1e-5f, s1.p, s));
    c1.A = h1.p; c1.lda = cin;
  }
  if (down) {
    CGD_TRY(u.ensure(h1p, npo * cin));
    CGD_TRY(u.ensure(xr, npo * cin));
    CGD_TRY(cgd_launch_resample2x_pair(ctx, 0, h1.p, cin, h1p.p, cin, x.p, x.ld, xr.p, cin, B, Ho, Wo, cin, 0.25f, s));
    c1.A = h1p.p; c1.lda = cin;
    skip_src = xr.p;
    skip_ld = cin;
  } else if (up) {
    CGD_TRY(u.ensure(xr, npo * cin));
    CGD_TRY(cgd_launch_upsample2x(ctx, x.p, x.ld, xr.p, cin, nullptr, 0, B, Ho, Wo, cin, 1.f, s));
    skip_src = xr.p;
    skip_ld = cin;
  }
  CGD_TRY(cgd_launch_gemm(ctx, c1, s));
  GemmParams c2;
  c2.A = h2.p; c2.lda = cout; c2.B = cw2f; c2.Bpk = cw2fp; c2.Bwk = wino_ready ? cw2wp : nullptr; c2.bwk_prec = wino_prec; c2.ldb = 9 * cout; c2.C = outp; c2.ldc = ldo; c2.bias = cb2;
  c2.M = (int)npo; c2.N = cout; c2.conv = 1; c2.H = Ho; c2.W = Wo; c2.Cin = cout;
  c2.defer = 1;
  c2.stats = 1;
  const bool fuse2 = cgd_conv_uses_hconv(ctx, c2);
  if (fuse2) {
    CGD_TRY(cgd_launch_gn_fwd(ctx, h2.p, cout, nullptr, 0, B, Ho * Wo, cout, g2, b2, u.emb_cur + emb_off, (int)u.emb_total, 1, 1e-5f,
                              s2.p, s));
    c2.gn_ab = cgd_gn_ab(s2.p, B, Ho * Wo, cout);
  } else {
    CGD_TRY(u.ensure(h3, npo * cout));
    CGD_TRY(cgd_launch_gn_fwd(ctx, h2.p, cout, h3.p, cout, B, Ho * Wo, cout, g2, b2, u.emb_cur + emb_off, (int)u.emb_total, 1, 1e-5f,
                              s2.p, s));
    c2.A = h3.p;
  }
  const float* R = skip_src;
  int ldr = skip_ld;
  if (skip_conv) {
    GemmParams sk;
    sk.A = skip_src; sk.lda = skip_ld; sk.B = skw; sk.ldb = cin; sk.C = outp; sk.ldc = ldo; sk.bias = skb;
    sk.M = (int)npo; sk.N = cout; sk.K = cin;
    sk.weight = 1;
    CGD_TRY(cgd_launch_gemm(ctx, sk, s));
    R = outp;
    ldr = ldo;
  }
  c2.R = R; c2.ldr = ldr;
  CGD_TRY(cgd_launch_gemm(ctx, c2, s));
  Hh = Ho; Ww = Wo;
  *o = TV{outp, ldo, cout};
  return 0;
}

int ResBlock::bwd(UNet& u, TV dout, TV* din, hipStream_t s) {
  cgd_ctx* ctx = u.ctx;
  const long npi = (long)B * H * W, npo = (long)B * Ho * Wo;
  CGD_TRY(u.ensure(d3, npo * cout));
  CGD_TRY(u.ensure(d2, npo * cout));
  CGD_TRY(u.ensure(d1, npo * cin));
  CGD_TRY(u.ensure(dx, npi * cin));
  GemmParams c2;
  c2.A = dout.p; c2.lda = dout.ld; c2.B = cw2d; c2.Bpk = cw2dp; c2.Bwk = wino_ready ? cw2wd : nullptr; c2.bwk_prec = wino_prec; c2.ldb = 9 * cout; c2.C = d3.p; c2.ldc = cout;
  c2.M = (int)npo; c2.N = cout; c2.conv = 1; c2.H = Ho; c2.W = Wo; c2.Cin = cout;
  c2.defer = 1;
  c2.gnb_x = h2.p; c2.gnb_ldx = cout; c2.gnb_coef = cgd_gn_coef(s2.p, B, Ho * Wo, cout); c2.gnb_act = 1;
  CGD_TRY(cgd_launch_gemm(ctx, c2, s));
  CGD_TRY(cgd_launch_gn_bwd(ctx, h2.p, cout, d3.p, cout, d2.p, cout, nullptr, 0, B, Ho * Wo, cout, 1, s2.p, s));
  const float* add = nullptr;
  int ldadd = 0;
  if (down || up) {
    add = dx.p; ldadd = cin;
  } else if (skip_conv) {
    GemmParams sk;
    sk.A = dout.p; sk.lda = dout.ld; sk.B = skwT; sk.ldb = cout; sk.C = dx.p; sk.ldc = cin;
    sk.M = (int)npo; sk.N = cin; sk.K = cout;
    sk.weight = 1;
    CGD_TRY(cgd_launch_gemm(ctx, sk, s));
    add = dx.p; ldadd = cin;
  } else {
    add = dout.p; ldadd = dout.ld;
  }
  GemmParams c1;
  c1.A = d2.p; c1.lda = cout; c1.B = cw1d; c1.Bpk = cw1dp; c1.Bwk = wino_ready ? cw1wd : nullptr; c1.bwk_prec = wino_prec; c1.ldb = 9 * cout; c1.C = d1.p; c1.ldc = cin;
  c1.M = (int)npo; c1.N = cin; c1.conv = 1; c1.H = Ho; c1.W = Wo; c1.Cin = cout;
  c1.defer = (up || down) ? 0 : 1;
  if (!up && !down) {
    c1.gnb_x = x.p; c1.gnb_ldx = x.ld; c1.gnb_coef = cgd_gn_coef(s1.p, B, H * W, cin); c1.gnb_act = 1;
  }
  CGD_TRY(cgd_launch_gemm(ctx, c1, s));
  const float* dh1 = d1.p;
  if (down) {
    CGD_TRY(u.ensure(d1f, npi * cin));
    CGD_TRY(cgd_launch_resample2x_pair(ctx, 1, d1.p, cin, d1f.p, cin, dout.p, dout.ld, dx.p, cin, B, H, W, cin, 0.25f, s));
    dh1 = d1f.p;
  } else if (up) {
    CGD_TRY(u.ensure(d1f, npi * cin));
    CGD_TRY(cgd_launch_resample2x_pair(ctx, 0, d1.p, cin, d1f.p, cin, dout.p, dout.ld, dx.p, cin, B, H, W, cin, 1.f, s));
    dh1 = d1f.p;
  }
  CGD_TRY(cgd_launch_gn_bwd(ctx, x.p, x.ld, dh1, cin, dx.p, cin, add, ldadd, B, H * W, cin, 1, s1.p, s, add_skip.p, add_skip.ld));
  *din = TV{dx.p, cin, cin};
  return 0;
}

int AttnBlock::fwd(UNet& u, TV xin, int Bn, int& H, int& W, TV* o, hipStream_t s) {
  cgd_ctx* ctx = u.ctx;
  B = Bn; T = H * W;
  x = xin;
  const long rows = (long)B * T;
  CGD_TRY(u.ensure(sc, cgd_gn_scratch_floats(B, T, C)));
  CGD_TRY(u.ensure(n, rows * C));
  CGD_TRY(u.ensure(qkv, rows * 3 * C));
  CGD_TRY(u.ensure(a, rows * C));
  if (!dst.p) CGD_TRY(u.ensure(out, rows * C));
  float* const outp = dst.p ? dst.p : out.p;
  const int ldo = dst.p ? dst.ld : C;
  CGD_TRY(cgd_launch_gn_fwd(ctx, x.p, x.ld, n.p, C, B, T, C, g, b, nullptr, 0, 0, 1e-5f, sc.p, s));
  GemmParams q;
  q.A = n.p; q.lda = C; q.B = qkvw; q.ldb = C; q.C = qkv.p; q.ldc = 3 * C; q.bias = qkvb; q.M = (int)rows; q.N = 3 * C; q.K = C;
  q.weight = 1;
  CGD_TRY(cgd_launch_gemm(ctx, q, s));
  CGD_TRY(u.attn_fwd(att, AttnShape{B, heads, T, d, C, legacy, 0}, qkv.p, 3 * C, a.p, C, s));
  GemmParams p;
  p.A = a.p; p.lda = C; p.B = pw; p.ldb = C; p.C = outp; p.ldc = ldo; p.bias = pb; p.R = x.p; p.ldr = x.ld; p.M = (int)rows; p.N = C;
  p.K = C;
  p.weight = 1;
  p.defer = 1;
  CGD_TRY(cgd_launch_gemm(ctx, p, s));
  *o = TV{outp, ldo, C};
  return 0;
}

int AttnBlock::bwd(UNet& u, TV dout, TV* din, hipStream_t s) {
  cgd_ctx* ctx = u.ctx;
  const long rows = (long)B * T;
  CGD_TRY(u.ensure(da, rows * C));
  CGD_TRY(u.ensure(dqkv, rows * 3 * C));
  CGD_TRY(u.ensure(dn, rows * C));
  CGD_TRY(u.ensure(dx, rows * C));
  GemmParams p;
  p.A = dout.p; p.lda = dout.ld; p.B = pwT; p.ldb = C; p.C = da.p; p.ldc = C; p.M = (int)rows; p.N = C; p.K = C;
  p.weight = 1;
  CGD_TRY(cgd_launch_gemm(ctx, p, s));
  CGD_TRY(u.attn_bwd(att, AttnShape{B, heads, T, d, C, legacy, 0}, qkv.p, 3 * C, da.p, C, dqkv.p, 3 * C, s));
  GemmParams q;
  q.A = dqkv.p; q.lda = 3 * C; q.B = qkvwT; q.ldb = 3 * C; q.C = dn.p; q.ldc = C; q.M = (int)rows; q.N = C; q.K = 3 * C;
  q.weight = 1;
  q.defer = 1;
  CGD_TRY(cgd_launch_gemm(ctx, q, s));
  CGD_TRY(cgd_launch_gn_bwd(ctx, x.p, x.ld, dn.p, C, dx.p, C, dout.p, dout.ld, B, T, C, 0, sc.p, s));
  *din = TV{dx.p, C, C};
  return 0;
}

int UNet::build() {
  const int mc = cfg.model_channels;
  if (cfg.in_channels != 3 || (!encoder_only && cfg.out_channels != 6 && cfg.out_channels != 3)) CGD_FAIL(ctx, "unet: in_channels must be 3, out_channels 3 or 6");
  if (cfg.n_mult < 1 || cfg.n_mult > 8) CGD_FAIL(ctx, "unet: bad channel_mult");
  if (cfg.n_att < 0 || cfg.n_att > 8) CGD_FAIL(ctx, "unet: at most 8 attention resolutions");
  if (mc <= 0 || mc % 32) CGD_FAIL(ctx, "unet: model_channels must be a positive multiple of 32 (GroupNorm32)");
  if (cfg.num_res_blocks < 1) CGD_FAIL(ctx, "unet: num_res_blocks must be >= 1");
  if (cfg.image_size <= 0 || cfg.image_size % (1 << (cfg.n_mult - 1))) CGD_FAIL(ctx, "unet: image_size must be divisible by 2^(levels-1)");
  if (cfg.num_classes < 0) CGD_FAIL(ctx, "unet: num_classes must be >= 0");
  if (cfg.num_head_channels == -1 ? cfg.num_heads <= 0 : cfg.num_head_channels <= 0) CGD_FAIL(ctx, "unet: num_heads / num_head_channels");
  for (int i = 0; i < cfg.n_mult; ++i) {
    const float w = cfg.channel_mult[i] * mc;
    const int wi = (int)w;
    if (!(w > 0.f) || (float)wi != w || wi % 32) CGD_FAIL(ctx, "unet: channel_mult * model_channels must be a positive multiple of 32 at every level");
    bool att = false;
    for (int a = 0; a < cfg.n_att; ++a) att = att || cfg.attention_ds[a] == (1 << i);
    if (att && (cfg.num_head_channels == -1 ? wi % cfg.num_heads : wi % cfg.num_head_channels))
      CGD_FAIL(ctx, "unet: the width of an attention level must be divisible by the head count / head width");
  }
  ted = mc * 4;
  add_param("time_embed.0.weight", (int64_t)ted * mc);
  add_param("time_embed.0.bias", ted);
  add_param("time_embed.2.weight", (int64_t)ted * ted);
  add_param("time_embed.2.bias", ted);
  if (cfg.num_classes > 0) add_param("label_emb.weight", (int64_t)cfg.num_classes * ted);

  auto is_att = [&](int ds) {
    for (int i = 0; i < cfg.n_att; ++i)
      if (cfg.attention_ds[i] == ds) return true;
// ... 509 lines not shown
```

### clip-guided-diffusion_amd/lib.py

```python
import ctypes as C
import os
import weakref

_HERE = os.path.dirname(os.path.abspath(__file__))
LIB_PATH = os.environ.get("CGD_LIB_PATH") or os.path.join(_HERE, "libcgd_mi355x.so")

F32P = C.POINTER(C.c_float)
vp = C.c_void_p
i32 = C.c_int
i64 = C.c_int64
f32 = C.c_float


class UNetConfig(C.Structure):
    _fields_ = [
        ("image_size", i32), ("model_channels", i32), ("num_res_blocks", i32), ("n_mult", i32),
        ("channel_mult", f32 * 8), ("n_att", i32), ("attention_ds", i32 * 8), ("num_classes", i32),
        ("num_heads", i32), ("num_head_channels", i32), ("use_new_attention_order", i32),
        ("in_channels", i32), ("out_channels", i32),
    ]


class ClassifierConfig(C.Structure):
    _fields_ = [
# ... 103 lines not shown
    "cgd_lpips_create": (i32, [vp, C.POINTER(vp)]),
    "cgd_lpips_destroy": (None, [vp]),
    "cgd_lpips_num_params": (i32, [vp]),
    "cgd_lpips_param_info": (i32, [vp, i32, C.c_char_p, i32, C.POINTER(i64)]),
    "cgd_lpips_set_param": (i32, [vp, C.c_char_p, vp, i64]),
    "cgd_lpips_finalize": (i32, [vp]),
    "cgd_lpips_set_reference": (i32, [vp, vp, i32, i32, i32, vp]),
    "cgd_lpips_loss_grad": (i32, [vp, vp, f32, vp, vp, i32, vp]),
    "cgd_lpips_debug_replay": (i32, [vp, C.POINTER(vp)]),
    "cgd_secondary_manifest": (i32, [MANIFEST_CB, vp]),
    "cgd_secondary_create": (i32, [vp, C.POINTER(vp)]),
    "cgd_secondary_destroy": (None, [vp]),
    "cgd_secondary_num_params": (i32, [vp]),
    "cgd_secondary_param_info": (i32, [vp, i32, C.c_char_p, i32, C.POINTER(i64)]),
    "cgd_secondary_set_param": (i32, [vp, C.c_char_p, vp, i64]),
    "cgd_secondary_finalize": (i32, [vp]),
    "cgd_secondary_forward": (i32, [vp, vp, vp, i32, i32, i32, vp, vp]),
    "cgd_secondary_forward_blend": (i32, [vp, vp, vp, i32, i32, i32, f32, vp, vp, vp]),
    "cgd_secondary_dgrad": (i32, [vp, vp, vp, vp]),
    "cgd_secondary_debug_replay": (i32, [vp, C.POINTER(vp)]),
    "cgd_secondary_head": (i32, [vp, vp, vp, vp, f32, vp, vp, i32, i32, i32, vp]),
    "cgd_secondary_combine": (i32, [vp, vp, vp, vp, vp, vp, vp, i32, i32, i32, f32, f32, f32, f32, f32, f32, vp]),
    "cgd_op_secondary_pack": (i32, [vp, vp, vp, vp, vp, i32, i32, i32, vp]),
    "cgd_op_bilinear_up2x": (i32, [vp, vp, i32, vp, i32, i32, i32, i32, i32, i32, vp]),
    "cgd_classifier_manifest": (i32, [C.POINTER(ClassifierConfig), MANIFEST_CB, vp]),
    "cgd_classifier_create": (i32, [vp, C.POINTER(ClassifierConfig), C.POINTER(vp)]),
    "cgd_classifier_destroy": (None, [vp]),
    "cgd_classifier_num_params": (i32, [vp]),
    "cgd_classifier_param_info": (i32, [vp, i32, C.c_char_p, i32, C.POINTER(i64)]),
    "cgd_classifier_set_param": (i32, [vp, C.c_char_p, vp, i64]),
    "cgd_classifier_finalize": (i32, [vp]),
    "cgd_classifier_forward": (i32, [vp, vp, vp, vp, vp, vp, i32, i32, i32, vp]),
    "cgd_classifier_dgrad": (i32, [vp, f32, vp, i32, vp]),
    "cgd_op_attnpool_scratch_floats": (i64, [i32, i32, i32, i32, i32]),
    "cgd_op_attnpool_fwd": (i32, [vp, vp, vp, vp, vp, vp, vp, vp, vp, vp, vp, vp, i32, i32, i32, i32, i32, vp]),
    "cgd_op_attnpool_bwd": (i32, [vp, vp, vp, vp, vp, f32, vp, vp, i32, i32, i32, i32, i32, vp]),
    "cgd_cutouts_fwd": (i32, [vp, vp, vp, vp, i32, i32, i32, i32, i32, i32, i32, vp]),
    "cgd_cutouts_bwd": (i32, [vp, vp, vp, vp, i32, i32, i32, i32, i32, i32, i32, i32, vp]),
    "cgd_cutouts_aug_fwd": (i32, [vp, vp, vp, vp, vp, vp, vp, i32, i32, i32, i32, i32, i32, i32, vp]),
    "cgd_cutouts_aug_bwd": (i32, [vp, vp, vp, vp, vp, vp, i32, i32, i32, i32, i32, i32, i32, i32, vp]),
    "cgd_cutouts_aug_scratch_floats": (i64, [i32, i32, i32, i32]),
    "cgd_op_aug_sample_map": (i32, [vp, i32, i32, vp, vp, vp]),
    "cgd_cutouts_resize_fwd": (i32, [vp, vp, vp, vp, vp, i32, i32, i32, i32, i32, i32, i32, vp]),
    "cgd_cutouts_resize_bwd": (i32, [vp, vp, vp, vp, vp, vp, i32, i32, i32, i32, i32, i32, i32, i32, vp]),
    "cgd_cutouts_resize_scratch_floats": (i64, [i32, i32, i32, i32]),
    "cgd_cutouts_resize_weights": (i32, [i32, i32, vp, vp, C.POINTER(i32)]),
    "cgd_spherical_loss": (i32, [vp, vp, vp, vp, vp, vp, i32, i32, i32, i32, f32, vp]),
    "cgd_directional_loss": (i32, [vp, vp, vp, vp, vp, vp, vp, i32, i32, i32, i32, i32, f32, i32, vp]),
    "cgd_pmv_blend": (i32, [vp, vp, vp, vp, vp, vp, vp, i32, i32, i32, C.POINTER(StepCoef), vp]),
    "cgd_guidance_part_blocks": (i32, [i32, i32, i32]),
    "cgd_guidance_combine": (i32, [vp, vp, vp, vp, vp, vp, vp, i32, i32, i32, C.POINTER(StepCoef), f32, f32, f32, vp]),
    "cgd_grad_finish": (i32, [vp, vp, vp, vp, vp, i32, i32, i32, vp]),
    "cgd_scalars": (i32, [vp, vp, i32, vp, vp, i32, i32, i32, i32, vp, vp]),
    "cgd_sample_update": (i32, [vp, vp, vp, vp, vp, vp, vp, vp, vp, vp, i32, i32, i32, C.POINTER(StepCoef), i32, vp]),
    "cgd_multistep_update": (i32, [vp, vp, vp, vp, vp, vp, vp, C.POINTER(vp), vp, vp, vp, i32, i32, i32, C.POINTER(StepCoef),
                                    C.POINTER(StepCoef), C.POINTER(Multistep), vp]),
    "cgd_dpmpp_update": (i32, [vp, vp, vp, vp, vp, vp, vp, vp, vp, vp, i32, i32, i32, C.POINTER(StepCoef), C.POINTER(Dpmpp), vp]),
    "cgd_abs_quantile_scratch_bytes": (i64, [i32, i64]),
    "cgd_abs_quantile_slice": (i32, []),
    "cgd_op_abs_quantile": (i32, [vp, vp, i32, i64, i64, f32, f32, f32, vp, vp, vp]),
    "cgd_dpmpp_threshold": (i32, [vp, vp, vp, vp, vp, vp, i32, i32, i32, C.POINTER(StepCoef), i64, f32, f32, f32, vp, vp, vp]),
    "cgd_dpmpp_update_thr": (i32, [vp, vp, vp, vp, vp, vp, vp, vp, vp, vp, i32, i32, i32, C.POINTER(StepCoef), C.POINTER(Dpmpp), vp]),
    "cgd_masked_merge": (i32, [vp, vp, vp, vp, vp, vp, vp, vp, i32, i32, i32, i32, i32, i32, C.POINTER(MaskCoef), vp]),
    "cgd_ddim_reverse_update": (i32, [vp, vp, vp, vp, vp, vp, vp, i32, i32, i32, i32, C.POINTER(ReverseCoef), vp]),
    "cgd_op_gemm": (i32, [vp, vp, i32, vp, i32, vp, i32, vp, vp, i32, i32, i32, i32, f32, i32, i32, vp]),
    "cgd_op_plan": (i32, [i32, i32, i32, i32, i32, i32, i32, i32, i32, i32, C.POINTER(i32)]),
    "cgd_op_pack_conv3x3_frag": (i32, [vp, vp, vp, i32, i32, i32, vp]),
    "cgd_set_hconv": (i32, [vp, i32, i32]),
    "cgd_op_conv3x3": (i32, [vp, vp, i32, vp, vp, vp, i32, vp, vp, i32, i32, i32, i32, i32, i32, i32, i32, i32, vp]),
    "cgd_op_pack_conv3x3_wino": (i32, [vp, vp, vp, i32, i32, i32, vp]),
    "cgd_op_conv3x3_wino": (i32, [vp, vp, i32, vp, vp, i32, vp, vp, i32, vp, i32, i32, i32, i32, i32, i32, vp]),
    "cgd_set_wino": (i32, [vp, i32, i32]),
    "cgd_op_conv3x3_wino_ex": (i32, [vp, vp, i32, vp, vp, i32, vp, vp, i32, vp, i32, i32, i32, i32, i32, i32, i32, vp, i32, vp, vp]),
    "cgd_op_new_pass": (i32, [vp]),
    "cgd_op_gn_record_merges": (i64, [vp]),
    "cgd_op_gn_stats_offset": (i64, [i32, i32, i32]),
    "cgd_op_wconv_schedule": (i32, [i32, i32, C.POINTER(i32)]),
    "cgd_op_mfma_peak": (i32, [vp, i32, C.POINTER(C.c_double), vp]),
    "cgd_op_conv_in": (i32, [vp, vp, vp, vp, vp, i32, i32, i32, i32, i32, vp]),
    "cgd_op_conv_thin_out": (i32, [vp, vp, i32, vp, vp, vp, i32, i32, i32, i32, i32, vp]),
    "cgd_op_gn_scratch_floats": (i64, [i32, i32, i32]),
    "cgd_op_gn_fwd": (i32, [vp, vp, i32, vp, i32, i32, i32, i32, vp, vp, vp, i32, f32, vp, vp]),
    "cgd_op_gn_bwd": (i32, [vp, vp, i32, vp, i32, vp, i32, vp, i32, i32, i32, i32, i32, vp, vp]),
    "cgd_op_ln_fwd": (i32, [vp, vp, vp, i32, i32, vp, vp, f32, vp, vp]),
    "cgd_op_ln_bwd": (i32, [vp, vp, vp, vp, i32, i32, vp, vp, vp]),
    "cgd_op_pool2x2": (i32, [vp, vp, vp, i32, i32, i32, i32, f32, vp]),
    "cgd_op_upsample2x": (i32, [vp, vp, vp, i32, i32, i32, i32, f32, vp]),
    "cgd_op_act": (i32, [vp, vp, vp, vp, i64, i32, vp]),
    "cgd_op_attn_buf_floats": (i64, [i32, i32, i32, i32, i32]),
    "cgd_op_attn_fwd": (i32, [vp, vp, vp, i32, i32, i32, i32, i32, C.POINTER(vp), vp]),
    "cgd_op_attn_bwd": (i32, [vp, vp, vp, vp, i32, i32, i32, i32, i32, C.POINTER(vp), vp]),
    "cgd_op_attn_fwd_causal": (i32, [vp, vp, vp, i32, i32, i32, i32, C.POINTER(vp), vp]),
    "cgd_op_attn_plan": (i32, [i32, i32, i32, i32, i32, i32, C.POINTER(i32)]),
}

EXPORTED_SYMBOLS = tuple(_SIGS)

_lib = None


def load():
    global _lib
    if _lib is None:
        if not os.path.isfile(LIB_PATH):
            raise RuntimeError(
                f"{LIB_PATH} not found: build it with `python -c 'import __graft_entry__ as g; g.build()'` "
                "(hipcc --offload-arch=gfx950). The MI355X path has no fallback.")
        lib = C.CDLL(LIB_PATH)
        for name, (res, args) in _SIGS.items():
            fn = getattr(lib, name)
            fn.restype = res
            fn.argtypes = args
        _lib = lib
    return _lib


class CgdError(RuntimeError):
    pass


class Context:

    def __init__(self, device=0, precision=None):
        import torch
        self.lib = load()
        if not torch.cuda.is_available():
            raise RuntimeError("cgd_mi355x needs an MI355X (gfx950) GPU visible to PyTorch-ROCm")
        h = vp()
        rc = self.lib.cgd_ctx_create(C.byref(h), int(device))
        if rc != 0:
            raise CgdError(f"cgd_ctx_create failed with status {rc} (is device {device} a gfx950?)")
        self.h = h
        self.device = int(device)
        self._nets = weakref.WeakSet()
        if precision is not None:
            self.set_precision(precision)
        tiles = os.environ.get("CGD_TILES")
        if tiles:
            large, small = (int(v) for v in tiles.split(","))
            self.check(self.lib.cgd_set_tiles(self.h, large, small))
        hg = os.environ.get("CGD_HGEMM")
        if hg:
            self.check(self.lib.cgd_set_hgemm(self.h, *(int(v) for v in hg.split(","))))
        hv = os.environ.get("CGD_HCONV_VAR")
        if hv:
            self.check(self.lib.cgd_set_hconv(self.h, 1 + 16 * int(hv), 256))

    def check(self, rc):
        if rc != 0:
            what = {-1: "HIP runtime error", -2: "invalid argument or state", -3: "NULL handle or pointer", -4: "not a gfx950 device"}.get(rc, "error")
            msg = self.lib.cgd_last_error(self.h).decode() if rc in (-1, -2) else ""
            raise CgdError(f"{what} (status {rc})" + (f": {msg}" if msg else ""))

    def set_precision(self, mode):
        mode = {"f32": 0, "bf16x3": 1, "bf16": 2}.get(mode, mode)
        self.check(self.lib.cgd_set_precision(self.h, int(mode)))

    @property
    def precision(self):
        return self.lib.cgd_get_precision(self.h)

    def stream(self):
        import torch
        return torch.cuda.current_stream(self.device).cuda_stream

    def close(self):
# ... 24 lines not shown
```

### clip-guided-diffusion_amd/ops.py

```python
import ctypes as C

import torch as th

from . import lib as L

_DEVICE_TYPE = "cuda"


def _s():
    return L.stream_ptr()


def _check(t, name):
    if not isinstance(t, th.Tensor):
        raise ValueError(f"{name}: expected a torch.Tensor, got {type(t).__name__}")
    if t.device.type != _DEVICE_TYPE:
        raise ValueError(f"{name}: expected a GPU tensor, got one on {t.device}")
    if t.dtype != th.float32:
        raise ValueError(f"{name}: expected float32, got {t.dtype}")


def _dense(t, name):
    if t is None:
        return None
# ... 54 lines not shown
    ctx.check(ctx.lib.cgd_op_pack_conv3x3_frag(ctx.h, pw, out.data_ptr(), co, ci, int(dgrad), _s()))
    return out


def conv3x3(ctx, x_nhwc, w_packed, bias=None, R=None, upsample_input=False, force_tile=0, splitk=1, w_frag=None):
    Bn, Hs, Ws, Cin = x_nhwc.shape
    H, W = (Hs * 2, Ws * 2) if upsample_input else (Hs, Ws)
    Cout = w_packed.shape[0]
    px, ldx = _rows(x_nhwc, "x")
    pw, pfrag, pbias = _dense(w_packed, "w_packed"), _dense(w_frag, "w_frag"), _dense(bias, "bias")
    pr, ldr = _rows(R, "R")
    y = th.empty((Bn, H, W, Cout), device=x_nhwc.device, dtype=th.float32)
    ctx.check(ctx.lib.cgd_op_conv3x3(ctx.h, px, ldx, pw, pfrag, y.data_ptr(), Cout, pbias, pr, ldr, Bn, H, W, Cin, Cout, int(upsample_input),
                                     force_tile, splitk, _s()))
    return y


def pack_conv3x3_wino(ctx, w, dgrad=False):
    co, ci = w.shape[:2]
    wc = w.contiguous().float()
    pw = _dense(wc, "w")
    out = th.empty(co * ci * 12, device=w.device, dtype=th.float32)
    ctx.check(ctx.lib.cgd_op_pack_conv3x3_wino(ctx.h, pw, out.data_ptr(), co, ci, int(dgrad), _s()))
    return out


def conv3x3_wino(ctx, x_nhwc, w_wino, cout, bias=None, R=None, upsample_input=False, gn_ab=None):
    Bn, Hs, Ws, Cin = x_nhwc.shape
    H, W = (Hs * 2, Ws * 2) if upsample_input else (Hs, Ws)
    px, ldx = _rows(x_nhwc, "x")
    pw, pbias, pab = _dense(w_wino, "w_wino"), _dense(bias, "bias"), _dense(gn_ab, "gn_ab")
    pr, ldr = _rows(R, "R")
    y = th.empty((Bn, H, W, cout), device=x_nhwc.device, dtype=th.float32)
    ctx.check(ctx.lib.cgd_op_conv3x3_wino(ctx.h, px, ldx, pw, y.data_ptr(), cout, pbias, pr, ldr, pab, Bn, H, W, Cin, cout, int(upsample_input),
                                          _s()))
    return y


def conv_in(ctx, x_nchw, w_packed, bias, cout):
    Bn, Cin, H, W = x_nchw.shape
    px, pw, pbias = _dense(x_nchw, "x"), _dense(w_packed, "w_packed"), _dense(bias, "bias")
    y = th.empty((Bn, H, W, cout), device=x_nchw.device, dtype=th.float32)
    ctx.check(ctx.lib.cgd_op_conv_in(ctx.h, px, pw, pbias, y.data_ptr(), Bn, H, W, Cin, cout, _s()))
    return y


def conv_thin_out(ctx, x_nhwc, w_packed, bias, cout):
    Bn, H, W, Cin = x_nhwc.shape
    px, ldx = _rows(x_nhwc, "x")
    pw, pbias = _dense(w_packed, "w_packed"), _dense(bias, "bias")
    y = th.empty((Bn, cout, H, W), device=x_nhwc.device, dtype=th.float32)
    ctx.check(ctx.lib.cgd_op_conv_thin_out(ctx.h, px, ldx, pw, pbias, y.data_ptr(), Bn, H, W, Cin, cout, _s()))
    return y


def gn_scratch(ctx, B, HW, C, device):
    n = ctx.lib.cgd_op_gn_scratch_floats(B, HW, C)
    return th.empty(n, device=device, dtype=th.float32)


def groupnorm_fwd(ctx, x, gamma, beta, film=None, act=1, eps=1e-5, scratch=None):
    B, HW, Cc = x.shape
    px, ldx = _rows(x, "x")
    pg, pb, pf = _dense(gamma, "gamma"), _dense(beta, "beta"), _dense(film, "film")
    if scratch is None:
        scratch = gn_scratch(ctx, B, HW, Cc, x.device)
    ps = _dense(scratch, "scratch")
    y = th.empty((B, HW, Cc), device=x.device, dtype=th.float32)
    ctx.check(ctx.lib.cgd_op_gn_fwd(ctx.h, px, ldx, y.data_ptr(), Cc, B, HW, Cc, pg, pb, pf, act, eps, ps, _s()))
    return y, scratch


def groupnorm_bwd(ctx, x, dz, scratch, act=1, add=None):
    B, HW, Cc = x.shape
    px, ldx = _rows(x, "x")
    pdz, lddz = _rows(dz, "dz")
    padd, ldadd = _rows(add, "add")
    ps = _dense(scratch, "scratch")
    dx = th.empty((B, HW, Cc), device=x.device, dtype=th.float32)
    ctx.check(ctx.lib.cgd_op_gn_bwd(ctx.h, px, ldx, pdz, lddz, dx.data_ptr(), Cc, padd, ldadd, B, HW, Cc, act, ps, _s()))
    return dx


def layernorm_fwd(ctx, x, gamma, beta, eps=1e-5):
    rows, Cc = x.shape
    px, pg, pb = _dense(x, "x"), _dense(gamma, "gamma"), _dense(beta, "beta")
    y = th.empty((rows, Cc), device=x.device, dtype=th.float32)
    stats = th.empty((rows, 2), device=x.device, dtype=th.float32)
    ctx.check(ctx.lib.cgd_op_ln_fwd(ctx.h, px, y.data_ptr(), rows, Cc, pg, pb, eps, stats.data_ptr(), _s()))
    return y, stats


def layernorm_bwd(ctx, x, dy, gamma, stats):
    rows, Cc = x.shape
    px, pdy, pg, pst = _dense(x, "x"), _dense(dy, "dy"), _dense(gamma, "gamma"), _dense(stats, "stats")
    dx = th.empty((rows, Cc), device=x.device, dtype=th.float32)
    ctx.check(ctx.lib.cgd_op_ln_bwd(ctx.h, px, pdy, dx.data_ptr(), rows, Cc, pg, pst, _s()))
    return dx


def pool2x2(ctx, x_nhwc, scale=0.25):
    B, H, W, Cc = x_nhwc.shape
    px = _dense(x_nhwc, "x")
    y = th.empty((B, H // 2, W // 2, Cc), device=x_nhwc.device, dtype=th.float32)
    ctx.check(ctx.lib.cgd_op_pool2x2(ctx.h, px, y.data_ptr(), B, H // 2, W // 2, Cc, scale, _s()))
    return y


def upsample2x(ctx, x_nhwc, scale=1.0):
    B, H, W, Cc = x_nhwc.shape
    px = _dense(x_nhwc, "x")
    y = th.empty((B, H * 2, W * 2, Cc), device=x_nhwc.device, dtype=th.float32)
    ctx.check(ctx.lib.cgd_op_upsample2x(ctx.h, px, y.data_ptr(), B, H * 2, W * 2, Cc, scale, _s()))
    return y


def act(ctx, x, kind, dy=None):
    px, pdy = _dense(x, "x"), _dense(dy, "dy")
    if dy is not None and dy.numel() != x.numel():
        raise ValueError(f"dy: {dy.numel()} elements, x has {x.numel()}")
    out = th.empty(x.shape, device=x.device, dtype=th.float32)
    ctx.check(ctx.lib.cgd_op_act(ctx.h, px, pdy, out.data_ptr(), x.numel(), kind, _s()))
    return out


class Attention:

    def __init__(self, ctx, nb, heads, T, d, legacy, device):
        self.ctx, self.nb, self.heads, self.T, self.d, self.legacy = ctx, nb, heads, T, d, int(legacy)
        self.bufs = [th.zeros(ctx.lib.cgd_op_attn_buf_floats(nb, heads, T, d, w), device=device, dtype=th.float32) for w in range(5)]
        self._arr = (C.c_void_p * 5)(*[b.data_ptr() for b in self.bufs])

    def forward(self, qkv):
        Cc = self.heads * self.d
        pq = _dense(qkv, "qkv")
        out = th.empty((self.nb * self.T, Cc), device=qkv.device, dtype=th.float32)
        self.ctx.check(self.ctx.lib.cgd_op_attn_fwd(self.ctx.h, pq, out.data_ptr(), self.nb, self.heads, self.T, self.d,
                                                    self.legacy, self._arr, _s()))
        return out

    def forward_causal(self, qkv):
        if self.legacy:
            raise ValueError("causal attention takes the [Q all heads | K | V] row layout (legacy=0)")
        Cc = self.heads * self.d
        pq = _dense(qkv, "qkv")
        out = th.empty((self.nb * self.T, Cc), device=qkv.device, dtype=th.float32)
        self.ctx.check(self.ctx.lib.cgd_op_attn_fwd_causal(self.ctx.h, pq, out.data_ptr(), self.nb, self.heads, self.T, self.d,
                                                           self._arr, _s()))
        return out

    def backward(self, qkv, dout):
        pq, pd = _dense(qkv, "qkv"), _dense(dout, "dout")
        dqkv = th.empty(qkv.shape, device=qkv.device, dtype=th.float32)
        self.ctx.check(self.ctx.lib.cgd_op_attn_bwd(self.ctx.h, pq, pd, dqkv.data_ptr(), self.nb, self.heads,
                                                    self.T, self.d, self.legacy, self._arr, _s()))
        return dqkv
```

### include/cgd_mi355x.h

```cpp
#ifndef CGD_MI355X_H
#define CGD_MI355X_H
#include <stdint.h>

#ifdef __cplusplus
extern "C" {
#endif

typedef struct cgd_ctx cgd_ctx;
typedef struct cgd_unet cgd_unet;
typedef struct cgd_vit cgd_vit;

enum { CGD_F32 = 0, CGD_BF16X3 = 1, CGD_BF16 = 2 };

int cgd_ctx_create(cgd_ctx** out, int device);
void cgd_ctx_destroy(cgd_ctx* ctx);
const char* cgd_last_error(cgd_ctx* ctx);
int cgd_set_precision(cgd_ctx* ctx, int mode);
int cgd_get_precision(cgd_ctx* ctx);
int64_t cgd_ctx_device_allocs(cgd_ctx* ctx);
const char* cgd_version(void);
int cgd_set_tiles(cgd_ctx* ctx, int large_tile, int small_tile);
int cgd_set_hgemm(cgd_ctx* ctx, int mode, int min_m, int min_chunks);
int cgd_profile(cgd_ctx* ctx, int enable);
int cgd_profile_read(cgd_ctx* ctx, double* out18);
// ... 197 lines not shown
  int order;
  float sigma;
  float dir;
} cgd_multistep;
int cgd_multistep_update(cgd_ctx* ctx, const float* x, const float* x_eval, const float* pred_xstart, const float* g,
                         const float* scalars, const float* noise, const float* const eps_hist[3], float* eps_out, float* sample,
                         float* pred_xstart_out, int B, int H, int W, const cgd_step_coef* k, const cgd_step_coef* k_step,
                         const cgd_multistep* m, void* stream);

typedef struct cgd_dpmpp {
  float c_x;
  float c_d;
  float c_r;
  float c_n;
} cgd_dpmpp;
int cgd_dpmpp_update(cgd_ctx* ctx, const float* x, const float* pred_xstart, const float* g, const float* scalars, const float* noise,
                     const float* x0_hist, float* x0c_out, float* sample, float* pred_xstart_out, int B, int H, int W,
                     const cgd_step_coef* k, const cgd_dpmpp* d, void* stream);

int64_t cgd_abs_quantile_scratch_bytes(int B, int64_t n);
int cgd_abs_quantile_slice(void);
int cgd_op_abs_quantile(cgd_ctx* ctx, const float* v, int B, int64_t n, int64_t k, float frac, float floor, float cap, float* out3,
                        void* scratch, void* stream);
int cgd_dpmpp_threshold(cgd_ctx* ctx, const float* x, const float* pred_xstart, const float* g, const float* scalars, float* x0c, int B,
                        int H, int W, const cgd_step_coef* k_coef, int64_t k, float frac, float floor, float cap, float* thr3, void* scratch,
                        void* stream);
int cgd_dpmpp_update_thr(cgd_ctx* ctx, const float* x, const float* pred_xstart, const float* x0c, const float* thr3, const float* noise,
                         const float* x0_hist, float* x0c_out, float* sample, float* pred_xstart_out, int B, int H, int W,
                         const cgd_step_coef* k_coef, const cgd_dpmpp* d, void* stream);

enum { CGD_MASK_PRED_XSTART = 1, CGD_MASK_N_KNOWN = 2, CGD_MASK_RENOISE = 4 };
typedef struct cgd_mask_coef {
  float sqrt_ab_prev;
  float sqrt_one_minus_ab_prev;
  float renoise_x;
  float renoise_n;
  int flags;
} cgd_mask_coef;
int cgd_masked_merge(cgd_ctx* ctx, float* sample, float* pred_xstart, const float* init, const float* mask, const float* n_known,
                     const float* n_re, float* x_re, int B, int H, int W, int init_batch, int mask_batch, int mask_channels,
                     const cgd_mask_coef* k, void* stream);

typedef struct cgd_reverse_coef {
  float sqrt_recip;
  float sqrt_recipm1;
  float sqrt_ab_next;
  float sqrt_one_minus_ab_next;
  float inv_sqrt_one_minus_ab_next;
} cgd_reverse_coef;
int cgd_ddim_reverse_update(cgd_ctx* ctx, const float* x, const float* model_out6, const float* init, float* x_next, float* pred_xstart,
                            float* noise_out, int B, int H, int W, int init_batch, const cgd_reverse_coef* k, void* stream);

int cgd_op_gemm(cgd_ctx* ctx, const float* A, int lda, const float* B, int ldb, float* C, int ldc, const float* bias, const float* R,
                int ldr, int M, int N, int K, float alpha, int force_tile, int splitk, void* stream);
int cgd_op_pack_conv3x3_frag(cgd_ctx* ctx, const float* w_torch, float* out , int Co, int Ci, int dgrad,
                             void* stream);
int cgd_op_plan(int conv, int M, int N, int K, int H, int W, int Cin, int weight, int precision, int num_cu, int* out4);
int cgd_set_hconv(cgd_ctx* ctx, int mode, int min_m);
int cgd_op_conv3x3(cgd_ctx* ctx, const float* x_nhwc, int ldx, const float* w_packed, const float* w_frag, float* y_nhwc, int ldy,
                   const float* bias, const float* R, int ldr, int Bn, int H, int W, int Cin, int Cout, int upsample_input, int force_tile,
                   int splitk, void* stream);
int cgd_op_pack_conv3x3_wino(cgd_ctx* ctx, const float* w_torch, float* out, int Co, int Ci, int dgrad, void* stream);
int cgd_op_conv3x3_wino(cgd_ctx* ctx, const float* x_nhwc, int ldx, const float* w_wino, float* y_nhwc, int ldy, const float* bias,
                        const float* R, int ldr, const float* gn_ab, int Bn, int H, int W, int Cin, int Cout, int upsample_input,
                        void* stream);
int cgd_set_wino(cgd_ctx* ctx, int mode, int min_m);
int cgd_op_conv3x3_wino_ex(cgd_ctx* ctx, const float* x_nhwc, int ldx, const float* w_wino, float* y_nhwc, int ldy, const float* bias,
                           const float* R, int ldr, const float* gn_ab, int Bn, int H, int W, int Cin, int Cout, int upsample_input,
                           int stats, const float* gnb_x, int gnb_ldx, const float* gnb_scratch, void* stream);
int cgd_op_new_pass(cgd_ctx* ctx);
int64_t cgd_op_gn_record_merges(cgd_ctx* ctx);
int64_t cgd_op_gn_stats_offset(int B, int HW, int C);
int cgd_op_wconv_schedule(int nb, int q, int* out7);
int cgd_op_mfma_peak(cgd_ctx* ctx, int iters, double* flop_out, void* stream);
int cgd_op_conv_in(cgd_ctx* ctx, const float* x_nchw, const float* w, const float* bias, float* y_nhwc, int Bn, int H, int W, int Cin,
                   int Cout, void* stream);
int cgd_op_conv_thin_out(cgd_ctx* ctx, const float* x_nhwc, int ldx, const float* w, const float* bias, float* y_nchw, int Bn, int H,
                         int W, int Cin, int Cout, void* stream);
int64_t cgd_op_gn_scratch_floats(int B, int HW, int C);
int cgd_op_gn_fwd(cgd_ctx* ctx, const float* x, int ldx, float* y, int ldy, int B, int HW, int C, const float* gamma,
                  const float* beta, const float* film, int act, float eps, float* scratch, void* stream);
int cgd_op_gn_bwd(cgd_ctx* ctx, const float* x, int ldx, const float* dz, int lddz, float* dx, int lddx, const float* add, int ldadd,
                  int B, int HW, int C, int act, float* scratch, void* stream);
int cgd_op_ln_fwd(cgd_ctx* ctx, const float* x, float* y, int rows, int C, const float* gamma, const float* beta, float eps,
                  float* stats, void* stream);
int cgd_op_ln_bwd(cgd_ctx* ctx, const float* x, const float* dy, float* dx, int rows, int C, const float* gamma, const float* stats,
                  void* stream);
int cgd_op_pool2x2(cgd_ctx* ctx, const float* in, float* out, int B, int Ho, int Wo, int C, float scale, void* stream);
int cgd_op_upsample2x(cgd_ctx* ctx, const float* in, float* out, int B, int Ho, int Wo, int C, float scale, void* stream);
int cgd_op_act(cgd_ctx* ctx, const float* x, const float* dy, float* out, int64_t n, int act, void* stream);
int64_t cgd_op_attn_buf_floats(int nb, int heads, int T, int d, int which);
int cgd_op_attn_fwd(cgd_ctx* ctx, const float* qkv, float* out, int nb, int heads, int T, int d, int legacy, float* bufs[5],
                    void* stream);
int cgd_op_attn_bwd(cgd_ctx* ctx, const float* qkv, const float* dout, float* dqkv, int nb, int heads, int T, int d, int legacy,
                    float* bufs[5], void* stream);
int cgd_op_attn_fwd_causal(cgd_ctx* ctx, const float* qkv, float* out, int nb, int heads, int T, int d, float* bufs[5], void* stream);
int cgd_op_attn_plan(int T, int d, int ldq, int ldo, int precision, int attn_flash, int* out2);

#ifdef __cplusplus
}
#endif
#endif
```

Measured before the change: 57.82 diffusion steps/sec.

## Fuse GroupNorm+SiLU into 2x2 pool and fold avg-pool backward into GN backward

```diff
diff --git a/clip-guided-diffusion_amd/csrc/capi.hip b/clip-guided-diffusion_amd/csrc/capi.hip
--- a/clip-guided-diffusion_amd/csrc/capi.hip
+++ b/clip-guided-diffusion_amd/csrc/capi.hip
@@ -41,6 +41,7 @@
   if (const char* e = getenv("CGD_TILE_ORDER")) ctx->tile_order = atoi(e);
   if (const char* e = getenv("CGD_FUSE_GN")) sscanf(e, "%d,%d,%d,%d", &ctx->fuse_gn, &ctx->fuse_gn_max_m, &ctx->fuse_gn_min_m, &ctx->fuse_gn_skip_m);
   if (const char* e = getenv("CGD_FUSE_ACT")) ctx->fuse_act = atoi(e);
+  if (const char* e = getenv("CGD_RESAMPLE_FUSED")) ctx->resample_fused = atoi(e);
   if (const char* e = getenv("CGD_HCONV_W8")) ctx->hconv_w8 = atoi(e);
   if (const char* e = getenv("CGD_ATTN_X3")) ctx->attn_x3 = atoi(e);
   if (const char* e = getenv("CGD_ATTN_FLASH")) ctx->attn_flash = atoi(e);
@@ -466,6 +467,29 @@
   CGD_NEED_CTX(ctx);
   return cgd_launch_gn_bwd(ctx, x, ldx, dz, lddz, dx, lddx, add, ldadd, B, HW, C, act, scratch, S(stream));
 }
+int cgd_op_gn_bwd_half(cgd_ctx* ctx, const float* x, int ldx, const float* dz, int lddz, float* dx, int lddx, const float* add, int ldadd,
+                       const float* add2, int ldadd2, int B, int H, int W, int C, int act, float dz_half, float add_half, float* scratch,
+                       void* stream) {
+  CGD_NEED_CTX(ctx);
+  return cgd_launch_gn_bwd(ctx, x, ldx, dz, lddz, dx, lddx, add, ldadd, B, H * W, C, act, scratch, S(stream), add2, ldadd2, W, dz_half, add_half);
+}
+int cgd_op_pool2x2_norm(cgd_ctx* ctx, const float* x, int ldx, const float* gn_scratch, int act, float* y_norm, float* y_pool, int B, int Ho,
+                        int Wo, int C, float scale, void* stream) {
+  CGD_NEED_CTX(ctx);
+  if (!gn_scratch) CGD_FAIL(ctx, "pool2x2_norm: needs the scratch of the cgd_op_gn_fwd over x");
+  return cgd_launch_pool2x2_norm_pair(ctx, x, ldx, cgd_gn_ab(gn_scratch, B, 4 * Ho * Wo, C), act, y_norm, C, y_pool, C, B, Ho, Wo, C, scale,
+                                      S(stream));
+}
+int cgd_op_conv3x3_deferred(cgd_ctx* ctx, const float* x, int ldx, const float* w, const float* w_frag, float* y, int ldy, const float* bias,
+                            int Bn, int H, int W, int Cin, int Cout, int force_tile, int splitk, void* stream) {
+  CGD_NEED_CTX(ctx);
+  GemmParams p;
+  p.Bpk = w_frag;
+  p.A = x; p.lda = ldx; p.B = w; p.ldb = 9 * Cin; p.C = y; p.ldc = ldy; p.bias = bias;
+  p.M = Bn * H * W; p.N = Cout; p.conv = 1; p.H = H; p.W = W; p.Cin = Cin; p.force_tile = force_tile; p.splitk = splitk;
+  p.defer = 1;
+  return cgd_launch_gemm(ctx, p, S(stream));
+}
 int cgd_op_ln_fwd(cgd_ctx* ctx, const float* x, float* y, int rows, int C, const float* gamma, const float* beta, float eps, float* stats,
                   void* stream) {
   CGD_NEED_CTX(ctx);
diff --git a/clip-guided-diffusion_amd/csrc/common.h b/clip-guided-diffusion_amd/csrc/common.h
--- a/clip-guided-diffusion_amd/csrc/common.h
+++ b/clip-guided-diffusion_amd/csrc/common.h
@@ -93,6 +93,7 @@
   int fuse_act = 1;
   int fuse_gn_skip_m = 0;
   int fuse_gn_max_m = 1 << 30, fuse_gn_min_m = 4096;
+  int resample_fused = 1;
   int fuse_gn = 1;
   int tile_order = 0;
   int hgemm_epi = 1;
diff --git a/clip-guided-diffusion_amd/csrc/elem.hip b/clip-guided-diffusion_amd/csrc/elem.hip
--- a/clip-guided-diffusion_amd/csrc/elem.hip
+++ b/clip-guided-diffusion_amd/csrc/elem.hip
@@ -84,6 +84,45 @@
   }
 }
 
+template <int ACT>
+__global__ __launch_bounds__(256) void pool2x2_norm_pair_kernel(const float* __restrict__ in, int ldi, const float* __restrict__ ab,
+                                                                float* __restrict__ outn, int ldon, float* __restrict__ outp, int ldop, int B,
+                                                                int Ho, int Wo, int C, float scale) {
+  const int cq = C >> 2;
+  const long total = (long)B * Ho * Wo * cq;
+  for (long i = (long)blockIdx.x * blockDim.x + threadIdx.x; i < total; i += (long)gridDim.x * blockDim.x) {
+    const int q = (int)(i % cq);
+    const long pix = i / cq;
+    const int x = (int)(pix % Wo);
+    const long t = pix / Wo;
+    const int y = (int)(t % Ho), b = (int)(t / Ho);
+    const long Wi = 2L * Wo;
+    const float* p00 = in + (((long)b * 2 * Ho + 2 * y) * Wi + 2 * x) * ldi + q * 4;
+    float4 v[4];
+    v[0] = *(const float4*)p00; v[1] = *(const float4*)(p00 + ldi);
+    v[2] = *(const float4*)(p00 + Wi * ldi); v[3] = *(const float4*)(p00 + Wi * ldi + ldi);
+    const float4* cf = (const float4*)(ab + ((long)b * C + q * 4) * 2);
+    const float4 c01 = cf[0], c23 = cf[1];
+    float4 n[4];
+#pragma unroll
+    for (int k = 0; k < 4; ++k) {
+      float4 o;
+      o.x = v[k].x * c01.x + c01.y;
+      o.y = v[k].y * c01.z + c01.w;
+      o.z = v[k].z * c23.x + c23.y;
+      o.w = v[k].w * c23.z + c23.w;
+      if (ACT == 1) {
+        o.x = o.x / (1.f + __expf(-o.x)); o.y = o.y / (1.f + __expf(-o.y)); o.z = o.z / (1.f + __expf(-o.z)); o.w = o.w / (1.f + __expf(-o.w));
+      }
+      n[k] = o;
+    }
+    *(float4*)(outn + pix * ldon + q * 4) = make_float4((n[0].x + n[1].x + n[2].x + n[3].x) * scale, (n[0].y + n[1].y + n[2].y + n[3].y) * scale,
+                                                        (n[0].z + n[1].z + n[2].z + n[3].z) * scale, (n[0].w + n[1].w + n[2].w + n[3].w) * scale);
+    *(float4*)(outp + pix * ldop + q * 4) = make_float4((v[0].x + v[1].x + v[2].x + v[3].x) * scale, (v[0].y + v[1].y + v[2].y + v[3].y) * scale,
+                                                        (v[0].z + v[1].z + v[2].z + v[3].z) * scale, (v[0].w + v[1].w + v[2].w + v[3].w) * scale);
+  }
+}
+
 __global__ __launch_bounds__(256) void copy2d_kernel(const float* __restrict__ a, int lda, const float* __restrict__ b, int ldb,
                                                      float* __restrict__ out, int ldo, long rows, int C) {
   const int cq = C >> 2;
@@ -247,6 +286,23 @@
   return 0;
 }
 
+int cgd_launch_pool2x2_norm_pair(cgd_ctx* ctx, const float* in, int ldi, const float* ab, int act, float* outn, int ldon, float* outp, int ldop,
+                                 int B, int Ho, int Wo, int C, float scale, hipStream_t s) {
+  CGD_TRY(cgd_sync_pending(ctx, s));
+  if ((C & 3) || ((ldi | ldon | ldop) & 3)) CGD_FAIL(ctx, "pool2x2_norm_pair: C and strides must be multiples of 4");
+  if (((uintptr_t)in | (uintptr_t)ab | (uintptr_t)outn | (uintptr_t)outp) & 15) CGD_FAIL(ctx, "pool2x2_norm_pair: in / ab / outputs must be 16-byte aligned");
+  if (!ab || (act != 0 && act != 1)) CGD_FAIL(ctx, "pool2x2_norm_pair: needs the norm's {a, b} coefficients and act 0 or 1 (SiLU)");
+  cgd_chanstats_invalidate(ctx, outn, (long)B * Ho * Wo, ldon, C);
+  cgd_chanstats_invalidate(ctx, outp, (long)B * Ho * Wo, ldop, C);
+  const dim3 grid(elem_grid((long)B * Ho * Wo * (C / 4)));
+  if (act)
+    CGD_LAUNCH((pool2x2_norm_pair_kernel<1>), grid, dim3(256), 0, s, in, ldi, ab, outn, ldon, outp, ldop, B, Ho, Wo, C, scale);
+  else
+    CGD_LAUNCH((pool2x2_norm_pair_kernel<0>), grid, dim3(256), 0, s, in, ldi, ab, outn, ldon, outp, ldop, B, Ho, Wo, C, scale);
+  CGD_HIP(ctx, hipGetLastError());
+  return 0;
+}
+
 int cgd_launch_copy2d(cgd_ctx* ctx, const float* a, int lda, const float* b, int ldb, float* out, int ldo, long rows, int C,
                       hipStream_t s) {
   CGD_TRY(cgd_sync_pending(ctx, s));
diff --git a/clip-guided-diffusion_amd/csrc/kernels.h b/clip-guided-diffusion_amd/csrc/kernels.h
--- a/clip-guided-diffusion_amd/csrc/kernels.h
+++ b/clip-guided-diffusion_amd/csrc/kernels.h
@@ -9,7 +9,7 @@
 size_t cgd_gn_stats_offset(int B, int HW, int C);
 int cgd_launch_gn_bwd(cgd_ctx* ctx, const float* x, int ldx, const float* dz, int lddz, float* dx, int lddx, const float* add,
                       int ldadd, int B, int HW, int C, int act, float* scratch, hipStream_t s, const float* add2 = nullptr,
-                      int ldadd2 = 0);
+                      int ldadd2 = 0, int half_w = 0, float dz_half = 0.f, float add_half = 0.f);
 int cgd_launch_ln_fwd(cgd_ctx* ctx, const float* x, int ldx, float* y, int ldy, int rows, int C, const float* gamma,
                       const float* beta, float eps, float* stats, hipStream_t s);
 int cgd_launch_ln_bwd(cgd_ctx* ctx, const float* x, int ldx, const float* dy, int lddy, float* dx, int lddx, const float* add,
@@ -21,6 +21,8 @@
                                int ldo1, int B, int Ho, int Wo, int C, float scale, hipStream_t s);
 int cgd_launch_upsample2x(cgd_ctx* ctx, const float* in, int ldi, float* out, int ldo, const float* add, int ldadd, int B, int Ho,
                           int Wo, int C, float scale, hipStream_t s);
+int cgd_launch_pool2x2_norm_pair(cgd_ctx* ctx, const float* in, int ldi, const float* ab, int act, float* outn, int ldon, float* outp, int ldop,
+                                 int B, int Ho, int Wo, int C, float scale, hipStream_t s);
 int cgd_launch_copy2d(cgd_ctx* ctx, const float* a, int lda, const float* b, int ldb, float* out, int ldo, long rows, int C,
                       hipStream_t s);
 int cgd_launch_concat2(cgd_ctx* ctx, const float* a, int lda, int Ca, const float* b, int ldb, int Cb, float* out, int ldo, long rows,
diff --git a/clip-guided-diffusion_amd/csrc/norm.hip b/clip-guided-diffusion_amd/csrc/norm.hip
--- a/clip-guided-diffusion_amd/csrc/norm.hip
+++ b/clip-guided-diffusion_amd/csrc/norm.hip
@@ -317,17 +317,33 @@
   }
 }
 
-template <int ACT>
+struct HalfMap {
+  int W = 0;
+  unsigned magic = 0;
+  float dzs = 0.f, adds = 0.f;
+};
+__device__ __forceinline__ int half_pix(int p, const HalfMap& hm, bool* owner) {
+  const int W = hm.W;
+  const int y = hm.magic ? (int)__umulhi((unsigned)p, hm.magic) : p / W, x = p - y * W;
+  *owner = !((y | x) & 1);
+  return (y >> 1) * (W >> 1) + (x >> 1);
+}
+__device__ __forceinline__ float4 scale4(float4 v, float s) { return make_float4(v.x * s, v.y * s, v.z * s, v.w * s); }
+
+template <int ACT, bool HALF>
 __global__ __launch_bounds__(256) void gn_bwd_partial_kernel(const float* __restrict__ x, int ldx, const float* dz, float* dzw,
                                                              int lddz, int HW, int C, int chunk, const float* __restrict__ coef,
-                                                             float* __restrict__ part , const SplitSrc src) {
+                                                             float* __restrict__ part , const SplitSrc src,
+                                                             const HalfMap hm) {
   __shared__ float lds_1[1024 * 4], lds_2[1024 * 4];
   __shared__ float red_1[256 * 4], red_2[256 * 4];
   const ColMap m = col_map(C);
   const int b = blockIdx.y, ck = blockIdx.x, nchunk = gridDim.x;
   const int p0 = ck * chunk, p1 = min(HW, p0 + chunk);
   const float* xb = x + ((long)b * HW) * ldx;
-  const float* db = dz + ((long)b * HW) * lddz;
+  const bool dzh = HALF && hm.dzs != 0.f;
+  const long drow0 = (long)b * (dzh ? HW >> 2 : HW);
+  const float* db = dz + drow0 * lddz;
   const int cpg = C / 32;
   for (int j = 0; j < MAXJ; ++j) {
     const int q = m.q0 + j * m.TQ;
@@ -342,12 +358,15 @@
        for (int u = 0; u < GN_U; ++u) {
          const int p = pb + u * m.rows, pc = p < p1 ? p : pb;
          vv[u] = *(const float4*)(xb + (long)pc * ldx + q * 4);
+         bool own = true;
+         const int pd = dzh ? half_pix(pc, hm, &own) : pc;
          if (src.n) {
-           dd[u] = split_load4(src, (long)b * HW + pc, q * 4);
-           if (p < p1) *(float4*)(dzw + ((long)b * HW + pc) * lddz + q * 4) = dd[u];
+           dd[u] = split_load4(src, drow0 + pd, q * 4);
+           if (p < p1 && own) *(float4*)(dzw + (drow0 + pd) * lddz + q * 4) = dd[u];
          } else {
-           dd[u] = *(const float4*)(db + (long)pc * lddz + q * 4);
+           dd[u] = *(const float4*)(db + (long)pd * lddz + q * 4);
          }
+         if (dzh) dd[u] = scale4(dd[u], hm.dzs);
        }
 #pragma unroll
        for (int u = 0; u < GN_U; ++u) {
@@ -473,19 +492,20 @@
 __device__ __forceinline__ void gn_st4_nt(float* p, const float4 o) {
   cgd_st16_nt(p, cgd_f32x4{o.x, o.y, o.z, o.w});
 }
-template <int ACT>
+template <int ACT, bool HALF>
 __global__ __launch_bounds__(256) void gn_bwd_apply_kernel(const float* __restrict__ x, int ldx, const float* __restrict__ dz,
                                                            int lddz, float* __restrict__ dx, int lddx, const float* __restrict__ add,
                                                            int ldadd, const float* __restrict__ add2, int ldadd2, int HW, int C, int chunk,
-                                                           const float* __restrict__ coef, const float* __restrict__ bcoef) {
+                                                           const float* __restrict__ coef, const float* __restrict__ bcoef, const HalfMap hm) {
   const ColMap m = col_map(C);
   if (!m.active) return;
   const int b = blockIdx.y;
   const int p0 = blockIdx.x * chunk, p1 = min(HW, p0 + chunk);
   const float* xb = x + ((long)b * HW) * ldx;
-  const float* db = dz + ((long)b * HW) * lddz;
+  const bool dzh = HALF && hm.dzs != 0.f, addh = HALF && hm.adds != 0.f;
+  const float* db = dz + ((long)b * (dzh ? HW >> 2 : HW)) * lddz;
   float* ob = dx + ((long)b * HW) * lddx;
-  const float* ab = add ? add + ((long)b * HW) * ldadd : nullptr;
+  const float* ab = add ? add + ((long)b * (addh ? HW >> 2 : HW)) * ldadd : nullptr;
   const float* ab2 = add2 ? add2 + ((long)b * HW) * ldadd2 : nullptr;
   for (int j = 0; j < MAXJ; ++j) {
     const int q = m.q0 + j * m.TQ;
@@ -500,8 +520,15 @@
      for (int u = 0; u < GN_U; ++u) {
        const int p = pb + u * m.rows, pc = p < p1 ? p : pb;
        vv[u] = gn_ld4_nt(xb + (long)pc * ldx + q * 4);
-       dd[u] = gn_ld4_nt(db + (long)pc * lddz + q * 4);
-       if (ab) aa[u] = gn_ld4_nt(ab + (long)pc * ldadd + q * 4);
+       if (HALF) {
+         bool own;
+         const int ph = half_pix(pc, hm, &own);
+         dd[u] = dzh ? scale4(*(const float4*)(db + (long)ph * lddz + q * 4), hm.dzs) : gn_ld4_nt(db + (long)pc * lddz + q * 4);
+         if (ab) aa[u] = addh ? scale4(*(const float4*)(ab + (long)ph * ldadd + q * 4), hm.adds) : gn_ld4_nt(ab + (long)pc * ldadd + q * 4);
+       } else {
+         dd[u] = gn_ld4_nt(db + (long)pc * lddz + q * 4);
+         if (ab) aa[u] = gn_ld4_nt(ab + (long)pc * ldadd + q * 4);
+       }
        if (ab2) {
          const float4 a2 = gn_ld4_nt(ab2 + (long)pc * ldadd2 + q * 4);
          if (ab) { aa[u].x += a2.x; aa[u].y += a2.y; aa[u].z += a2.z; aa[u].w += a2.w; } else aa[u] = a2;
@@ -886,11 +913,11 @@
   }
 }
 
-template <int ACT, int VEC, bool CACHE>
+template <int ACT, int VEC, bool CACHE, bool HALF>
 __global__ __launch_bounds__(GS_NT) void gn_small_bwd_kernel(const float* __restrict__ x, int ldx, const float* dz, float* dzw, int lddz,
                                                              float* dx, int lddx, const float* add, int ldadd, const float* add2, int ldadd2,
                                                              int HW, int C, int lg, const float* __restrict__ stats,
-                                                             const float* __restrict__ coef, const SplitSrc src) {
+                                                             const float* __restrict__ coef, const SplitSrc src, const HalfMap hm) {
   typedef typename VecT<VEC>::T V;
   __shared__ float red[GS_NT / 64];
   const int g = blockIdx.x, b = blockIdx.y, cpg = C / 32, cq = cpg / VEC, n = HW * cpg;
@@ -898,12 +925,14 @@
   const bool act_q = q < cq;
   const int qc = act_q ? q : 0;
   const float* xg = x + (long)b * HW * ldx + g * cpg + qc * VEC;
-  const float* dg = dz + (long)b * HW * lddz + g * cpg + qc * VEC;
-  float* dwg = dzw + (long)b * HW * lddz + g * cpg + qc * VEC;
-  const long row0 = (long)b * HW;
+  const bool dzh = HALF && hm.dzs != 0.f, addh = HALF && hm.adds != 0.f;
+  const long row0 = (long)b * (dzh ? HW >> 2 : HW);
+  const float* dg = dz + row0 * lddz + g * cpg + qc * VEC;
+  float* dwg = dzw + row0 * lddz + g * cpg + qc * VEC;
   const int col = g * cpg + qc * VEC;
   float* og = dx + (long)b * HW * lddx + g * cpg + qc * VEC;
-  const float* ag = add ? add + (long)b * HW * ldadd + g * cpg + qc * VEC : nullptr;
+  const float* ag = add ? add + (long)b * (addh ? HW >> 2 : HW) * ldadd + g * cpg + qc * VEC : nullptr;
+  bool own;
   const float* ag2 = add2 ? add2 + (long)b * HW * ldadd2 + g * cpg + qc * VEC : nullptr;
   const float mean = stats[((long)b * 32 + g) * 2], rstd = stats[((long)b * 32 + g) * 2 + 1];
   float a[VEC], bb[VEC], gc[VEC];
@@ -922,7 +951,9 @@
       const int p = r + it * rows;
       if (act_q && p < HW) {
         xc[it] = *(const V*)(xg + (long)p * ldx);
-        dc[it] = src.n ? split_load<VEC>(src, row0 + p, col) : *(const V*)(dg + (long)p * lddz);
+        const int pd = dzh ? half_pix(p, hm, &own) : p;
+        dc[it] = src.n ? split_load<VEC>(src, row0 + pd, col) : *(const V*)(dg + (long)pd * lddz);
+        if (dzh) dc[it] *= hm.dzs;
       }
     }
 #pragma unroll
@@ -948,12 +979,14 @@
       for (int u = 0; u < GS_U; ++u) {
         const int p = p0 + u * rows, pc = p < HW ? p : r;
         xv[u] = *(const V*)(xg + (long)pc * ldx);
+        const int pd = dzh ? half_pix(pc, hm, &own) : pc;
         if (src.n) {
-          dv[u] = split_load<VEC>(src, row0 + pc, col);
-          if (p < HW) *(V*)(dwg + (long)pc * lddz) = dv[u];
+          dv[u] = split_load<VEC>(src, row0 + pd, col);
+          if (p < HW && !dzh) *(V*)(dwg + (long)pc * lddz) = dv[u];
         } else {
-          dv[u] = *(const V*)(dg + (long)pc * lddz);
-        }
+          dv[u] = *(const V*)(dg + (long)pd * lddz);
+        }
+        if (dzh) dv[u] *= hm.dzs;
       }
 #pragma unroll
       for (int u = 0; u < GS_U; ++u) {
@@ -980,7 +1013,10 @@
 #pragma unroll
     for (int it = 0; it < 4; ++it) {
       const int p = r + it * rows;
-      if (ag && p < HW) av[it] = *(const V*)(ag + (long)p * ldadd);
+      if (ag && p < HW) {
+        av[it] = *(const V*)(ag + (long)(addh ? half_pix(p, hm, &own) : p) * ldadd);
+        if (addh) av[it] *= hm.adds;
+      }
       if (ag2 && p < HW) {
         const V a2 = *(const V*)(ag2 + (long)p * ldadd2);
         if (ag) av[it] += a2; else av[it] = a2;
@@ -1008,8 +1044,14 @@
     for (int u = 0; u < GS_U; ++u) {
       const int p = p0 + u * rows, pc = p < HW ? p : r;
       xv[u] = *(const V*)(xg + (long)pc * ldx);
-      dv[u] = *(const V*)(dg + (long)pc * lddz);
-      if (ag) av[u] = *(const V*)(ag + (long)pc * ldadd);
+      const int ph = HALF ? half_pix(pc, hm, &own) : pc;
+      const int pd = dzh ? ph : pc;
+      dv[u] = (dzh && src.n) ? split_load<VEC>(src, row0 + pd, col) : *(const V*)(dg + (long)pd * lddz);
+      if (dzh) dv[u] *= hm.dzs;
+      if (ag) {
+        av[u] = *(const V*)(ag + (long)(addh ? ph : pc) * ldadd);
+        if (addh) av[u] *= hm.adds;
+      }
       if (ag2) {
         const V a2 = *(const V*)(ag2 + (long)pc * ldadd2);
         if (ag) av[u] += a2; else av[u] = a2;
@@ -1056,7 +1098,7 @@
 template <int ACT>
 void launch_gn_small_bwd(const float* x, int ldx, const float* dz, int lddz, float* dx, int lddx, const float* add, int ldadd,
                          const float* add2, int ldadd2, int B, int HW, int C, const float* stats, const float* coef, hipStream_t s,
-                         const SplitSrc& src) {
+                         const SplitSrc& src, const HalfMap& hm) {
   const int cpg = C / 32;
   const bool v4 = !(cpg & 3) && !(ldx & 3) && !(lddz & 3) && !(lddx & 3) && !(ldadd & 3) && !(ldadd2 & 3) &&
                   !(((uintptr_t)x | (uintptr_t)dz | (uintptr_t)dx | (uintptr_t)add | (uintptr_t)add2) & 15) && !(src.n && ((src.N | src.ldr) & 3));
@@ -1064,11 +1106,17 @@
   int lg = 0;
   while ((1 << lg) < cq) ++lg;
   const bool cache = (long)HW <= 4L * (GS_NT >> lg) && !getenv("CGD_GN_NOCACHE");
-#define GN_SB(V_, C_) CGD_LAUNCH((gn_small_bwd_kernel<ACT, V_, C_>), dim3(32, B), dim3(GS_NT), 0, s, x, ldx, dz, (float*)dz, lddz, dx, lddx, add, ldadd, add2, ldadd2, HW, C, lg, stats, coef, src)
-  if (v4) {
-    if (cache) GN_SB(4, true); else GN_SB(4, false);
+#define GN_SB(V_, C_, H_) CGD_LAUNCH((gn_small_bwd_kernel<ACT, V_, C_, H_>), dim3(32, B), dim3(GS_NT), 0, s, x, ldx, dz, (float*)dz, lddz, dx, lddx, add, ldadd, add2, ldadd2, HW, C, lg, stats, coef, src, hm)
+  if (hm.W) {
+    if (v4) {
+      if (cache) GN_SB(4, true, true); else GN_SB(4, false, true);
+    } else {
+      if (cache) GN_SB(1, true, true); else GN_SB(1, false, true);
+    }
+  } else if (v4) {
+    if (cache) GN_SB(4, true, false); else GN_SB(4, false, false);
   } else {
-    if (cache) GN_SB(1, true); else GN_SB(1, false);
+    if (cache) GN_SB(1, true, false); else GN_SB(1, false, false);
   }
 #undef GN_SB
 }
@@ -1190,8 +1238,16 @@
 }
 
 int cgd_launch_gn_bwd(cgd_ctx* ctx, const float* x, int ldx, const float* dz, int lddz, float* dx, int lddx, const float* add,
-                      int ldadd, int B, int HW, int C, int act, float* scratch, hipStream_t s, const float* add2, int ldadd2) {
+                      int ldadd, int B, int HW, int C, int act, float* scratch, hipStream_t s, const float* add2, int ldadd2, int half_w,
+                      float dz_half, float add_half) {
   if (C % 32 || C > 4096) CGD_FAIL(ctx, "groupnorm backward: C must be a multiple of 32 and <= 4096");
+  HalfMap hm;
+  if (dz_half != 0.f || (add && add_half != 0.f)) {
+    if (half_w <= 0 || (half_w & 1) || HW % half_w || ((HW / half_w) & 1)) CGD_FAIL(ctx, "groupnorm backward: half-resolution operands need an even map (half_w = its width)");
+    hm.W = half_w; hm.dzs = dz_half; hm.adds = add ? add_half : 0.f;
+    if ((long)HW * half_w <= (1L << 32)) hm.magic = (unsigned)(((1UL << 32) + half_w - 1) / half_w);
+  }
+  const long dz_rows = (long)B * (hm.dzs != 0.f ? HW / 4 : HW);
   if (HW > GN_SMALL_HW && (((ldx | lddz | lddx | (add ? ldadd : 0) | (add2 ? ldadd2 : 0)) & 3) ||
                            (((uintptr_t)x | (uintptr_t)dz | (uintptr_t)dx | (uintptr_t)add | (uintptr_t)add2) & 15)))
     CGD_FAIL(ctx, "groupnorm backward: above the single-launch size, row strides must be multiples of 4 and x / dz / dx / add 16-byte aligned");
@@ -1199,19 +1255,20 @@
   float *part, *stats, *coef, *bcoef;
   gn_layout(scratch, B, HW, C, &chunk, &nchunk, &part, &stats, &coef, &bcoef);
   SplitSrc src;
-  if (!((HW > GN_SMALL_HW || ctx->defer_mode >= 2) && cgd_take_pending(ctx, dz, (long)B * HW, C, lddz, s, &src))) CGD_TRY(cgd_flush_pending(ctx, s));
+  if (!((HW > GN_SMALL_HW || ctx->defer_mode >= 2) && cgd_take_pending(ctx, dz, dz_rows, C, lddz, s, &src))) CGD_TRY(cgd_flush_pending(ctx, s));
   if (src.n && (((src.N | src.ldr) & 3) || ((uintptr_t)src.ws & 15) || ((uintptr_t)src.R & 15) || ((uintptr_t)src.bias & 15)) && HW > GN_SMALL_HW) {
-    ctx->pending.valid = true; ctx->pending.src = src; ctx->pending.C = (float*)dz; ctx->pending.ldc = lddz; ctx->pending.M = B * HW; ctx->pending.stream = s;
+    ctx->pending.valid = true; ctx->pending.src = src; ctx->pending.C = (float*)dz; ctx->pending.ldc = lddz; ctx->pending.M = (int)dz_rows; ctx->pending.stream = s;
     CGD_TRY(cgd_flush_pending(ctx, s));
     src = SplitSrc();
   }
   ProfRec pr;
-  CGD_TRY(cgd_prof_begin(ctx, &pr, CGD_PROF_GN, (12.0 + (add ? 4.0 : 0.0) + (add2 ? 4.0 : 0.0) + (src.n ? 4.0 * src.n : 0.0)) * B * HW * C, s));
+  const double dzb = hm.dzs != 0.f ? 0.25 : 1.0, addb = hm.adds != 0.f ? 0.25 : 1.0;
+  CGD_TRY(cgd_prof_begin(ctx, &pr, CGD_PROF_GN, (8.0 + 4.0 * dzb + (add ? 4.0 * addb : 0.0) + (add2 ? 4.0 : 0.0) + (src.n ? 4.0 * src.n * dzb : 0.0)) * B * HW * C, s));
   if (HW <= GN_SMALL_HW) {
     if (act)
-      launch_gn_small_bwd<1>(x, ldx, dz, lddz, dx, lddx, add, ldadd, add2, ldadd2, B, HW, C, stats, coef, s, src);
+      launch_gn_small_bwd<1>(x, ldx, dz, lddz, dx, lddx, add, ldadd, add2, ldadd2, B, HW, C, stats, coef, s, src, hm);
     else
-      launch_gn_small_bwd<0>(x, ldx, dz, lddz, dx, lddx, add, ldadd, add2, ldadd2, B, HW, C, stats, coef, s, src);
+      launch_gn_small_bwd<0>(x, ldx, dz, lddz, dx, lddx, add, ldadd, add2, ldadd2, B, HW, C, stats, coef, s, src, hm);
     CGD_TRY(cgd_prof_stamp(ctx, &pr, s));
     cgd_prof_push(ctx, &pr);
     CGD_HIP(ctx, hipGetLastError());
@@ -1219,7 +1276,7 @@
     return 0;
   }
   ChanSrc cs;
-  const bool merged = !src.n && !(HW & 127) && (ctx->gn_epi & 2) && cgd_chanstats_find(ctx, dz, lddz, (long)B * HW, C, s, &cs, 1) && cs.n0 == C;
+  const bool merged = !src.n && hm.dzs == 0.f && !(HW & 127) && (ctx->gn_epi & 2) && cgd_chanstats_find(ctx, dz, lddz, (long)B * HW, C, s, &cs, 1) && cs.n0 == C;
   cgd_chanstats_invalidate(ctx, dx, (long)B * HW, lddx, C);
   if (merged) {
     ++ctx->gn_record_merges;
@@ -1227,18 +1284,22 @@
     while ((1 << lg) < C / 32) ++lg;
     CGD_LAUNCH(gn_bwd_coef_ch_kernel, dim3(32, B), dim3(256), 0, s, cs.p0, HW / 128, lg, stats, coef, C, HW, bcoef);
   } else {
-    if (act) {
-      CGD_LAUNCH((gn_bwd_partial_kernel<1>), dim3(nchunk, B), dim3(256), 0, s, x, ldx, dz, (float*)dz, lddz, HW, C, chunk, coef, part, src);
+#define GN_BP(A_, H_) CGD_LAUNCH((gn_bwd_partial_kernel<A_, H_>), dim3(nchunk, B), dim3(256), 0, s, x, ldx, dz, (float*)dz, lddz, HW, C, chunk, coef, part, src, hm)
+    if (hm.W) {
+      if (act) GN_BP(1, true); else GN_BP(0, true);
     } else {
-      CGD_LAUNCH((gn_bwd_partial_kernel<0>), dim3(nchunk, B), dim3(256), 0, s, x, ldx, dz, (float*)dz, lddz, HW, C, chunk, coef, part, src);
-    }
+      if (act) GN_BP(1, false); else GN_BP(0, false);
+    }
+#undef GN_BP
     CGD_LAUNCH(gn_bwd_coef_kernel, dim3(32, B), dim3(256), 0, s, part, nchunk, stats, coef, C, HW, bcoef);
   }
-  if (act) {
-    CGD_LAUNCH((gn_bwd_apply_kernel<1>), dim3(nchunk, B), dim3(256), 0, s, x, ldx, dz, lddz, dx, lddx, add, ldadd, add2, ldadd2, HW, C, chunk, coef, bcoef);
+#define GN_BA(A_, H_) CGD_LAUNCH((gn_bwd_apply_kernel<A_, H_>), dim3(nchunk, B), dim3(256), 0, s, x, ldx, dz, lddz, dx, lddx, add, ldadd, add2, ldadd2, HW, C, chunk, coef, bcoef, hm)
+  if (hm.W) {
+    if (act) GN_BA(1, true); else GN_BA(0, true);
   } else {
-    CGD_LAUNCH((gn_bwd_apply_kernel<0>), dim3(nchunk, B), dim3(256), 0, s, x, ldx, dz, lddz, dx, lddx, add, ldadd, add2, ldadd2, HW, C, chunk, coef, bcoef);
-  }
+    if (act) GN_BA(1, false); else GN_BA(0, false);
+  }
+#undef GN_BA
   CGD_TRY(cgd_prof_stamp(ctx, &pr, s));
   cgd_prof_push(ctx, &pr);
   CGD_HIP(ctx, hipGetLastError());
diff --git a/clip-guided-diffusion_amd/csrc/unet.hip b/clip-guided-diffusion_amd/csrc/unet.hip
--- a/clip-guided-diffusion_amd/csrc/unet.hip
+++ b/clip-guided-diffusion_amd/csrc/unet.hip
@@ -149,9 +149,12 @@
   c1.stats = 1;
   c1.A = x.p; c1.lda = x.ld;
   const bool fuse1 = !down && cgd_conv_uses_hconv(ctx, c1);
+  const bool pool_fused = down && ctx->resample_fused;
   const float* skip_src = x.p;
   int skip_ld = x.ld;
-  if (fuse1) {
+  if (pool_fused) {
+    CGD_TRY(cgd_launch_gn_fwd(ctx, x.p, x.ld, nullptr, 0, B, H * W, cin, g1, b1, nullptr, 0, 1, 1e-5f, s1.p, s));
+  } else if (fuse1) {
     CGD_TRY(cgd_launch_gn_fwd(ctx, x.p, x.ld, nullptr, 0, B, H * W, cin, g1, b1, nullptr, 0, 1, 1e-5f, s1.p, s));
     c1.gn_ab = cgd_gn_ab(s1.p, B, H * W, cin);
   } else {
@@ -162,7 +165,10 @@
   if (down) {
     CGD_TRY(u.ensure(h1p, npo * cin));
     CGD_TRY(u.ensure(xr, npo * cin));
-    CGD_TRY(cgd_launch_resample2x_pair(ctx, 0, h1.p, cin, h1p.p, cin, x.p, x.ld, xr.p, cin, B, Ho, Wo, cin, 0.25f, s));
+    if (pool_fused)
+      CGD_TRY(cgd_launch_pool2x2_norm_pair(ctx, x.p, x.ld, cgd_gn_ab(s1.p, B, H * W, cin), 1, h1p.p, cin, xr.p, cin, B, Ho, Wo, cin, 0.25f, s));
+    else
+      CGD_TRY(cgd_launch_resample2x_pair(ctx, 0, h1.p, cin, h1p.p, cin, x.p, x.ld, xr.p, cin, B, Ho, Wo, cin, 0.25f, s));
     c1.A = h1p.p; c1.lda = cin;
     skip_src = xr.p;
     skip_ld = cin;
@@ -223,7 +229,10 @@
   CGD_TRY(cgd_launch_gn_bwd(ctx, h2.p, cout, d3.p, cout, d2.p, cout, nullptr, 0, B, Ho * Wo, cout, 1, s2.p, s));
   const float* add = nullptr;
   int ldadd = 0;
-  if (down || up) {
+  const bool half = down && ctx->resample_fused;
+  if (half) {
+    add = dout.p; ldadd = dout.ld;
+  } else if (down || up) {
     add = dx.p; ldadd = cin;
   } else if (skip_conv) {
     GemmParams sk;
@@ -238,22 +247,19 @@
   GemmParams c1;
   c1.A = d2.p; c1.lda = cout; c1.B = cw1d; c1.Bpk = cw1dp; c1.Bwk = wino_ready ? cw1wd : nullptr; c1.bwk_prec = wino_prec; c1.ldb = 9 * cout; c1.C = d1.p; c1.ldc = cin;
   c1.M = (int)npo; c1.N = cin; c1.conv = 1; c1.H = Ho; c1.W = Wo; c1.Cin = cout;
-  c1.defer = (up || down) ? 0 : 1;
+  c1.defer = (up || (down && !half)) ? 0 : 1;
   if (!up && !down) {
     c1.gnb_x = x.p; c1.gnb_ldx = x.ld; c1.gnb_coef = cgd_gn_coef(s1.p, B, H * W, cin); c1.gnb_act = 1;
   }
   CGD_TRY(cgd_launch_gemm(ctx, c1, s));
   const float* dh1 = d1.p;
-  if (down) {
+  if (up || (down && !half)) {
     CGD_TRY(u.ensure(d1f, npi * cin));
-    CGD_TRY(cgd_launch_resample2x_pair(ctx, 1, d1.p, cin, d1f.p, cin, dout.p, dout.ld, dx.p, cin, B, H, W, cin, 0.25f, s));
+    CGD_TRY(cgd_launch_resample2x_pair(ctx, down ? 1 : 0, d1.p, cin, d1f.p, cin, dout.p, dout.ld, dx.p, cin, B, H, W, cin, down ? 0.25f : 1.f, s));
     dh1 = d1f.p;
-  } else if (up) {
-    CGD_TRY(u.ensure(d1f, npi * cin));
-    CGD_TRY(cgd_launch_resample2x_pair(ctx, 0, d1.p, cin, d1f.p, cin, dout.p, dout.ld, dx.p, cin, B, H, W, cin, 1.f, s));
-    dh1 = d1f.p;
-  }
-  CGD_TRY(cgd_launch_gn_bwd(ctx, x.p, x.ld, dh1, cin, dx.p, cin, add, ldadd, B, H * W, cin, 1, s1.p, s, add_skip.p, add_skip.ld));
+  }
+  CGD_TRY(cgd_launch_gn_bwd(ctx, x.p, x.ld, dh1, cin, dx.p, cin, add, ldadd, B, H * W, cin, 1, s1.p, s, add_skip.p, add_skip.ld, half ? W : 0,
+                            half ? 0.25f : 0.f, half ? 0.25f : 0.f));
   *din = TV{dx.p, cin, cin};
   return 0;
 }
diff --git a/clip-guided-diffusion_amd/lib.py b/clip-guided-diffusion_amd/lib.py
--- a/clip-guided-diffusion_amd/lib.py
+++ b/clip-guided-diffusion_amd/lib.py
@@ -209,6 +209,9 @@
     "cgd_op_gn_scratch_floats": (i64, [i32, i32, i32]),
     "cgd_op_gn_fwd": (i32, [vp, vp, i32, vp, i32, i32, i32, i32, vp, vp, vp, i32, f32, vp, vp]),
     "cgd_op_gn_bwd": (i32, [vp, vp, i32, vp, i32, vp, i32, vp, i32, i32, i32, i32, i32, vp, vp]),
+    "cgd_op_gn_bwd_half": (i32, [vp, vp, i32, vp, i32, vp, i32, vp, i32, vp, i32, i32, i32, i32, i32, i32, f32, f32, vp, vp]),
+    "cgd_op_pool2x2_norm": (i32, [vp, vp, i32, vp, i32, vp, vp, i32, i32, i32, i32, f32, vp]),
+    "cgd_op_conv3x3_deferred": (i32, [vp, vp, i32, vp, vp, vp, i32, vp, i32, i32, i32, i32, i32, i32, i32, vp]),
     "cgd_op_ln_fwd": (i32, [vp, vp, vp, i32, i32, vp, vp, f32, vp, vp]),
     "cgd_op_ln_bwd": (i32, [vp, vp, vp, vp, i32, i32, vp, vp, vp]),
     "cgd_op_pool2x2": (i32, [vp, vp, vp, i32, i32, i32, i32, f32, vp]),
diff --git a/clip-guided-diffusion_amd/ops.py b/clip-guided-diffusion_amd/ops.py
--- a/clip-guided-diffusion_amd/ops.py
+++ b/clip-guided-diffusion_amd/ops.py
@@ -160,6 +160,39 @@
     return dx
 
 
+def groupnorm_bwd_half(ctx, x_nhwc, dz, scratch, act=1, add=None, add2=None, dz_half=0.25, add_half=0.25):
+    B, H, W, Cc = x_nhwc.shape
+    px, ldx = _rows(x_nhwc, "x")
+    pdz, lddz = _rows(dz, "dz")
+    padd, ldadd = _rows(add, "add")
+    padd2, ldadd2 = _rows(add2, "add2")
+    ps = _dense(scratch, "scratch")
+    dx = th.empty((B, H, W, Cc), device=x_nhwc.device, dtype=th.float32)
+    ctx.check(ctx.lib.cgd_op_gn_bwd_half(ctx.h, px, ldx, pdz, lddz, dx.data_ptr(), Cc, padd, ldadd, padd2, ldadd2, B, H, W, Cc, act, dz_half,
+                                         add_half if add is not None else 0.0, ps, _s()))
+    return dx
+
+
+def pool2x2_norm(ctx, x_nhwc, scratch, act=1, scale=0.25):
+    B, H, W, Cc = x_nhwc.shape
+    px, ldx = _rows(x_nhwc, "x")
+    ps = _dense(scratch, "scratch")
+    yn = th.empty((B, H // 2, W // 2, Cc), device=x_nhwc.device, dtype=th.float32)
+    yp = th.empty_like(yn)
+    ctx.check(ctx.lib.cgd_op_pool2x2_norm(ctx.h, px, ldx, ps, act, yn.data_ptr(), yp.data_ptr(), B, H // 2, W // 2, Cc, scale, _s()))
+    return yn, yp
+
+
+def conv3x3_deferred(ctx, x_nhwc, w_packed, splitk, bias=None, force_tile=0, w_frag=None):
+    Bn, H, W, Cin = x_nhwc.shape
+    Cout = w_packed.shape[0]
+    px, ldx = _rows(x_nhwc, "x")
+    pw, pfrag, pbias = _dense(w_packed, "w_packed"), _dense(w_frag, "w_frag"), _dense(bias, "bias")
+    y = th.empty((Bn, H, W, Cout), device=x_nhwc.device, dtype=th.float32)
+    ctx.check(ctx.lib.cgd_op_conv3x3_deferred(ctx.h, px, ldx, pw, pfrag, y.data_ptr(), Cout, pbias, Bn, H, W, Cin, Cout, force_tile, splitk, _s()))
+    return y
+
+
 def layernorm_fwd(ctx, x, gamma, beta, eps=1e-5):
     rows, Cc = x.shape
     px, pg, pb = _dense(x, "x"), _dense(gamma, "gamma"), _dense(beta, "beta")
diff --git a/include/cgd_mi355x.h b/include/cgd_mi355x.h
--- a/include/cgd_mi355x.h
+++ b/include/cgd_mi355x.h
@@ -303,6 +303,13 @@
                   const float* beta, const float* film, int act, float eps, float* scratch, void* stream);
 int cgd_op_gn_bwd(cgd_ctx* ctx, const float* x, int ldx, const float* dz, int lddz, float* dx, int lddx, const float* add, int ldadd,
                   int B, int HW, int C, int act, float* scratch, void* stream);
+int cgd_op_gn_bwd_half(cgd_ctx* ctx, const float* x, int ldx, const float* dz, int lddz, float* dx, int lddx, const float* add, int ldadd,
+                       const float* add2, int ldadd2, int B, int H, int W, int C, int act, float dz_half, float add_half, float* scratch,
+                       void* stream);
+int cgd_op_pool2x2_norm(cgd_ctx* ctx, const float* x, int ldx, const float* gn_scratch, int act, float* y_norm, float* y_pool, int B, int Ho,
+                        int Wo, int C, float scale, void* stream);
+int cgd_op_conv3x3_deferred(cgd_ctx* ctx, const float* x, int ldx, const float* w, const float* w_frag, float* y, int ldy, const float* bias,
+                            int Bn, int H, int W, int Cin, int Cout, int force_tile, int splitk, void* stream);
 int cgd_op_ln_fwd(cgd_ctx* ctx, const float* x, float* y, int rows, int C, const float* gamma, const float* beta, float eps,
                   float* stats, void* stream);
 int cgd_op_ln_bwd(cgd_ctx* ctx, const float* x, const float* dy, float* dx, int rows, int C, const float* gamma, const float* stats,
```

After: 58.05 diffusion steps/sec (median of 6 runs). No clear change (+0.4%).
